# bogus2000/anytime-3D-reconstruction

Measured on AMD Instinct MI355X. Metric: 32^3 voxel reconstructions/sec at batch=256; IoU delta vs reference, higher is better.
Workload: dtype bf16

## Files before the change

### anytime-3d-reconstruction_amd/csrc/conv_direct.hip

```cpp
#include "direct_common.h"

namespace {

constexpr int CD_CIN = 64, CD_COUT = 128;
constexpr int CD_RB = CD_CIN * 2;
constexpr int CD_PIECES = 51;
constexpr int CD_TILE = CD_PIECES * 1024;
constexpr int CD_WST = CD_COUT * 128;
constexpr int CD_NST = 3;
constexpr int CD_RING = 2 * CD_TILE;
constexpr int CD_DUMMY = CD_RING + CD_NST * CD_WST;
constexpr int CD_LDS = CD_DUMMY + 1024;
constexpr int CD_SP = CD_COUT * 2 + 16;

__global__ __launch_bounds__(512, 1) void conv_direct_kernel(const __bf16 *__restrict__ x, const __bf16 *__restrict__ w,
                                                             const float *__restrict__ scale, const float *__restrict__ shift,
                                                             void *__restrict__ y, int dout_log2, unsigned x_bytes, unsigned w_bytes,
                                                             int act, int out_fp8) {
    extern __shared__ __attribute__((aligned(16))) char smem[];
    const int tid = threadIdx.x, lane = tid & 63;
    const int wave = __builtin_amdgcn_readfirstlane(tid >> 6);
    const int wm = wave >> 1, wn = wave & 1;
    const int lo = dout_log2, no = 1 << lo, li = lo + 1, n = 1 << li;

    const VvDirectBox box = vv_direct_box(no);
    const int b = box.b, od0 = box.od0, oh0 = box.oh0, ow0 = box.ow0;

    const u32x4 rsx = vv_make_rsrc(x, x_bytes), rsw = vv_make_rsrc(w, w_bytes);
    const unsigned lds0 = (unsigned)(unsigned long long)(lptr_t)smem;

    auto issue_x = [&](int q, int slot) {
        const int piece = slot * 8 + wave;
        const int rl = piece * 8 + (lane >> 3);
        const int zd = rl / 81, rem = rl - zd * 81, jh = rem / 9, jw = rem - jh * 9;
        const int g = (lane & 7) ^ (jw & 7);
        const int id = 2 * (od0 + zd) + ((q >> 2) & 1) - 1, ih = 2 * (oh0 + jh) + ((q >> 1) & 1) - 1, iw = 2 * (ow0 + jw) + (q & 1) - 1;
        const bool ok = q < 8 && rl < 405 && (unsigned)id < (unsigned)n && (unsigned)ih < (unsigned)n && (unsigned)iw < (unsigned)n;
        const unsigned vo = ok ? (unsigned)((((((b << li) + id) << li) + ih) << li) + iw) * CD_RB + g * 16 : 0xFFFFFFF0u;
        const unsigned dst = piece < CD_PIECES ? lds0 + (q & 1) * CD_TILE + piece * 1024 : lds0 + CD_DUMMY;
        vv_dma16(rsx, vo, dst);
    };
    auto issue_w = [&](int c) {
        const int q = c >> 3, a = c & 7;
        const int td = 2 * ((a >> 2) & 1) + ((q >> 2) & 1), th = 2 * ((a >> 1) & 1) + ((q >> 1) & 1), tw = 2 * (a & 1) + (q & 1);
        const int t = (td * 4 + th) * 4 + tw;
        const unsigned st = lds0 + CD_RING + (c % CD_NST) * CD_WST;
#pragma unroll
        for (int i = 0; i < 2; ++i) {
            const int row = (wave * 2 + i) * 8 + (lane >> 3);
            const int g = (lane & 7) ^ ((row >> 1) & 7);
            const unsigned vo = c < 64 ? (unsigned)row * (64 * CD_RB) + t * CD_RB + g * 16 : 0xFFFFFFF0u;
            vv_dma16(rsw, vo, st + (wave * 2 + i) * 1024);
        }
    };

#pragma unroll 1
    for (int s = 0; s < 7; ++s) issue_x(0, s);
    issue_w(0);
    issue_w(1);
    issue_w(2);
    vv_wait_vm<0>();
    __syncthreads();

    const int fr = lane & 31, fh = lane >> 5;
    const int rl0 = wm * 81 + (fr >> 3) * 9 + (fr & 7);
    unsigned xo[2][4], wo[4];
#pragma unroll
    for (int aw = 0; aw < 2; ++aw)
#pragma unroll
        for (int ks = 0; ks < 4; ++ks) xo[aw][ks] = lds0 + rl0 * CD_RB + (((ks * 2 + fh) ^ (((fr & 7) + aw) & 7)) << 4);
#pragma unroll
    for (int ks = 0; ks < 4; ++ks) wo[ks] = lds0 + CD_RING + (wn * 64 + fr) * 128 + (((ks * 2 + fh) ^ ((fr >> 1) & 7)) << 4);

    f32x16 acc[2][2];
#pragma unroll
    for (int i = 0; i < 2; ++i)
#pragma unroll
        for (int j = 0; j < 2; ++j)
#pragma unroll
            for (int e = 0; e < 16; ++e) acc[i][j][e] = 0.f;

#define CD_LDFRAG(F, XA, XOFF, WA)                                                                                              \
    asm volatile("ds_read_b128 %0, %4 offset:%6\n\tds_read_b128 %1, %4 offset:%7\n\tds_read_b128 %2, %5\n\tds_read_b128 %3, %5 offset:4096" \
                 : "=&v"(F[0]), "=&v"(F[1]), "=&v"(F[2]), "=&v"(F[3])                                                           \
                 : "v"(XA), "v"(WA), "n"(XOFF), "n"((XOFF) + 4 * 9 * CD_RB)                                                    \
                 : "memory")
#define CD_WAITFRAG(F, N) asm volatile("s_waitcnt lgkmcnt(%4)" : "+v"(F[0]), "+v"(F[1]), "+v"(F[2]), "+v"(F[3]) : "n"(N) : "memory")
#define CD_MFMA4(F)                                                                                                             \
    do {                                                                                                                        \
        _Pragma("unroll") for (int nt = 0; nt < 2; ++nt) _Pragma("unroll") for (int mt = 0; mt < 2; ++mt)                       \
            acc[nt][mt] = __builtin_amdgcn_mfma_f32_32x32x16_bf16(*reinterpret_cast<const bf16x8 *>(&F[2 + nt]),                \
                                                                  *reinterpret_cast<const bf16x8 *>(&F[mt]), acc[nt][mt], 0, 0, 0); \
        __builtin_amdgcn_sched_barrier(0);                                                                                      \
    } while (0)

    u32x4 P[4], Q[4];
    CD_LDFRAG(P, xo[0][0], 0, wo[0]);

#pragma unroll 1
    for (int q = 0; q < 8; ++q) {
        const unsigned tsel = (q & 1) * CD_TILE, tnext = ((q + 1) & 1) * CD_TILE;
        auto tap = [&](auto a_c) {
            constexpr int A = decltype(a_c)::value;
            constexpr int AW = A & 1, TO = (((A >> 2) & 1) * 81 + ((A >> 1) & 1) * 9 + AW) * CD_RB;
            constexpr int AN = (A + 1) & 7, AWN = AN & 1, TON = (((AN >> 2) & 1) * 81 + ((AN >> 1) & 1) * 9 + AWN) * CD_RB;
            const int c = q * 8 + A;
            const unsigned wsel = (c % CD_NST) * CD_WST, wnext = ((c + 1) % CD_NST) * CD_WST;
            CD_LDFRAG(Q, xo[AW][1] + tsel, TO, wo[1] + wsel);
            CD_WAITFRAG(P, 4);
            CD_MFMA4(P);
            CD_LDFRAG(P, xo[AW][2] + tsel, TO, wo[2] + wsel);
            CD_WAITFRAG(Q, 4);
            CD_MFMA4(Q);
            CD_LDFRAG(Q, xo[AW][3] + tsel, TO, wo[3] + wsel);
            CD_WAITFRAG(P, 4);
            CD_MFMA4(P);
            CD_WAITFRAG(Q, 0);
            vv_wait_vm<(A == 0 || A == 7) ? 2 : 3>();
            __syncthreads();
            if (A < 7) issue_x(q + 1, A);
            issue_w(c + 3);
            CD_LDFRAG(P, xo[AWN][0] + (A == 7 ? tnext : tsel), TON, wo[0] + wnext);
            CD_MFMA4(Q);
        };
        tap(std::integral_constant<int, 0>{});
        tap(std::integral_constant<int, 1>{});
        tap(std::integral_constant<int, 2>{});
        tap(std::integral_constant<int, 3>{});
        tap(std::integral_constant<int, 4>{});
        tap(std::integral_constant<int, 5>{});
        tap(std::integral_constant<int, 6>{});
        tap(std::integral_constant<int, 7>{});
    }
    CD_WAITFRAG(P, 0);
    vv_wait_vm<0>();
    __syncthreads();

    char *stage = smem;
    f32x4 scv[2][4], shv[2][4];
#pragma unroll
    for (int nt = 0; nt < 2; ++nt)
#pragma unroll
        for (int g = 0; g < 4; ++g) { scv[nt][g] = f32x4{1.f, 1.f, 1.f, 1.f}; shv[nt][g] = f32x4{0.f, 0.f, 0.f, 0.f}; }
    if (scale) {
#pragma unroll
        for (int nt = 0; nt < 2; ++nt)
#pragma unroll
            for (int g = 0; g < 4; ++g) scv[nt][g] = *reinterpret_cast<const f32x4 *>(scale + wn * 64 + nt * 32 + 8 * g + 4 * fh);
    }
    if (shift) {
#pragma unroll
        for (int nt = 0; nt < 2; ++nt)
#pragma unroll
            for (int g = 0; g < 4; ++g) shv[nt][g] = *reinterpret_cast<const f32x4 *>(shift + wn * 64 + nt * 32 + 8 * g + 4 * fh);
    }
    auto fill = VV_DIRECT_FILL32(CD_SP, wn * 64);
    auto with_out = [&](auto act_c) {
        if (out_fp8) fill(act_c, std::true_type{});
        else fill(act_c, std::false_type{});
    };
    VV_WITH_ACT(act, with_out);
    __syncthreads();
    vv_direct_store_box<512, CD_SP, CD_COUT, CD_COUT>(stage, y, box, lo, tid, out_fp8);
}

__global__ __launch_bounds__(512, 1) void conv_direct16_kernel(const __bf16 *__restrict__ x, const __bf16 *__restrict__ w,
                                                             const float *__restrict__ scale, const float *__restrict__ shift,
                                                             void *__restrict__ y, int dout_log2, unsigned x_bytes, unsigned w_bytes,
                                                             int act, int out_fp8) {
    extern __shared__ __attribute__((aligned(16))) char smem[];
    const int tid = threadIdx.x, lane = tid & 63;
    const int wave = __builtin_amdgcn_readfirstlane(tid >> 6);
    const int wm = wave >> 1, wn = wave & 1;
    const int lo = dout_log2, no = 1 << lo, li = lo + 1, n = 1 << li;

    const VvDirectBox box = vv_direct_box(no);
    const int b = box.b, od0 = box.od0, oh0 = box.oh0, ow0 = box.ow0;

    const u32x4 rsx = vv_make_rsrc(x, x_bytes), rsw = vv_make_rsrc(w, w_bytes);
    const unsigned lds0 = (unsigned)(unsigned long long)(lptr_t)smem;

    auto issue_x = [&](int q, int slot) {
        const int piece = slot * 8 + wave;
        const int rl = piece * 8 + (lane >> 3);
        const int zd = rl / 81, rem = rl - zd * 81, jh = rem / 9, jw = rem - jh * 9;
        const int g = (lane & 7) ^ ((2 * jw) & 7);
        const int id = 2 * (od0 + zd) + ((q >> 2) & 1) - 1, ih = 2 * (oh0 + jh) + ((q >> 1) & 1) - 1, iw = 2 * (ow0 + jw) + (q & 1) - 1;
        const bool ok = q < 8 && rl < 405 && (unsigned)id < (unsigned)n && (unsigned)ih < (unsigned)n && (unsigned)iw < (unsigned)n;
        const unsigned vo = ok ? (unsigned)((((((b << li) + id) << li) + ih) << li) + iw) * CD_RB + g * 16 : 0xFFFFFFF0u;
        const unsigned dst = piece < CD_PIECES ? lds0 + (q & 1) * CD_TILE + piece * 1024 : lds0 + CD_DUMMY;
        vv_dma16(rsx, vo, dst);
    };
    auto issue_w = [&](int c) {
        const int q = c >> 3, a = c & 7;
        const int td = 2 * ((a >> 2) & 1) + ((q >> 2) & 1), th = 2 * ((a >> 1) & 1) + ((q >> 1) & 1), tw = 2 * (a & 1) + (q & 1);
        const int t = (td * 4 + th) * 4 + tw;
        const unsigned st = lds0 + CD_RING + (c % CD_NST) * CD_WST;
#pragma unroll
        for (int i = 0; i < 2; ++i) {
            const int row = (wave * 2 + i) * 8 + (lane >> 3);
            const int g = (lane & 7) ^ ((row >> 1) & 7);
            const unsigned vo = c < 64 ? (unsigned)row * (64 * CD_RB) + t * CD_RB + g * 16 : 0xFFFFFFF0u;
            vv_dma16(rsw, vo, st + (wave * 2 + i) * 1024);
        }
    };

#pragma unroll 1
    for (int s = 0; s < 7; ++s) issue_x(0, s);
    issue_w(0);
    issue_w(1);
    issue_w(2);
    vv_wait_vm<0>();
    __syncthreads();

    const int r = lane & 15, kq = lane >> 4;
    const int rl0 = wm * 81 + (r >> 3) * 9 + (r & 7);
    unsigned xo[2][2], wo[2];
#pragma unroll
    for (int aw = 0; aw < 2; ++aw)
#pragma unroll
        for (int ks = 0; ks < 2; ++ks) xo[aw][ks] = lds0 + rl0 * CD_RB + (((ks * 4 + kq) ^ ((2 * ((r & 7) + aw)) & 7)) << 4);
#pragma unroll
    for (int ks = 0; ks < 2; ++ks) wo[ks] = lds0 + CD_RING + (wn * 64 + r) * 128 + (((ks * 4 + kq) ^ ((r >> 1) & 7)) << 4);

    f32x4 acc[4][4];
#pragma unroll
    for (int i = 0; i < 4; ++i)
#pragma unroll
        for (int j = 0; j < 4; ++j) acc[i][j] = f32x4{0.f, 0.f, 0.f, 0.f};

#define CD16_LD(F, XA, XOFF, WA)                                                                                                    \
    asm volatile("ds_read_b128 %0, %8 offset:%10\n\tds_read_b128 %1, %8 offset:%11\n\tds_read_b128 %2, %8 offset:%12\n\t"         \
                 "ds_read_b128 %3, %8 offset:%13\n\tds_read_b128 %4, %9\n\tds_read_b128 %5, %9 offset:2048\n\t"                   \
                 "ds_read_b128 %6, %9 offset:4096\n\tds_read_b128 %7, %9 offset:6144"                                               \
                 : "=&v"(F[0]), "=&v"(F[1]), "=&v"(F[2]), "=&v"(F[3]), "=&v"(F[4]), "=&v"(F[5]), "=&v"(F[6]), "=&v"(F[7])            \
                 : "v"(XA), "v"(WA), "n"(XOFF), "n"((XOFF) + 2304), "n"((XOFF) + 4608), "n"((XOFF) + 6912)                          \
                 : "memory")
#define CD16_WAIT(F, N)                                                                                                             \
    asm volatile("s_waitcnt lgkmcnt(%8)"                                                                                            \
                 : "+v"(F[0]), "+v"(F[1]), "+v"(F[2]), "+v"(F[3]), "+v"(F[4]), "+v"(F[5]), "+v"(F[6]), "+v"(F[7])                    \
                 : "n"(N)                                                                                                           \
                 : "memory")
#define CD16_SB __builtin_amdgcn_sched_barrier(0)
#define CD16_RD(D, A, OFF) asm volatile("ds_read_b128 %0, %1 offset:%2" : "=&v"(D) : "v"(A), "n"(OFF) : "memory")
#define CD16_MF(F, COT, CT)                                                                                                         \
    acc[COT][CT] = __builtin_amdgcn_mfma_f32_16x16x32_bf16(*reinterpret_cast<const bf16x8 *>(&F[4 + COT]),                          \
                                                           *reinterpret_cast<const bf16x8 *>(&F[CT]), acc[COT][CT], 0, 0, 0)

    u32x4 P[8], Q[8];
    CD16_LD(P, xo[0][0], 0, wo[0]);

#pragma unroll 1
    for (int q = 0; q < 8; ++q) {
        const unsigned tsel = (q & 1) * CD_TILE, tnext = ((q + 1) & 1) * CD_TILE;
        auto tap = [&](auto a_c) {
            constexpr int A = decltype(a_c)::value;
            constexpr int AW = A & 1, TO = (((A >> 2) & 1) * 81 + ((A >> 1) & 1) * 9 + AW) * CD_RB;
            constexpr int AN = (A + 1) & 7, AWN = AN & 1, TON = (((AN >> 2) & 1) * 81 + ((AN >> 1) & 1) * 9 + AWN) * CD_RB;
            const int c = q * 8 + A;
            const unsigned wsel = (c % CD_NST) * CD_WST, wnext = ((c + 1) % CD_NST) * CD_WST;
            const unsigned xq = xo[AW][1] + tsel, wq = wo[1] + wsel;
            CD16_WAIT(P, 0);
            CD16_SB;
            CD16_MF(P, 0, 0); CD16_MF(P, 0, 1); CD16_SB; CD16_RD(Q[0], xq, TO); CD16_RD(Q[4], wq, 0); CD16_SB;
            CD16_MF(P, 0, 2); CD16_MF(P, 0, 3); CD16_SB; CD16_RD(Q[1], xq, TO + 2304); CD16_RD(Q[5], wq, 2048); CD16_SB;
            CD16_MF(P, 1, 0); CD16_MF(P, 1, 1); CD16_SB; CD16_RD(Q[2], xq, TO + 4608); CD16_RD(Q[6], wq, 4096); CD16_SB;
            CD16_MF(P, 1, 2); CD16_MF(P, 1, 3); CD16_SB; CD16_RD(Q[3], xq, TO + 6912); CD16_RD(Q[7], wq, 6144); CD16_SB;
            CD16_MF(P, 2, 0); CD16_MF(P, 2, 1); CD16_MF(P, 2, 2); CD16_MF(P, 2, 3);
            CD16_MF(P, 3, 0); CD16_MF(P, 3, 1); CD16_MF(P, 3, 2); CD16_MF(P, 3, 3);
            CD16_SB;
            CD16_WAIT(Q, 0);
            vv_wait_vm<(A == 0 || A == 7) ? 2 : 3>();
            __syncthreads();
            CD16_SB;
            CD16_MF(Q, 0, 0); CD16_MF(Q, 0, 1);
            if (A < 7) issue_x(q + 1, A);
            CD16_MF(Q, 0, 2); CD16_MF(Q, 0, 3);
            issue_w(c + 3);
            const unsigned xp = xo[AWN][0] + (A == 7 ? tnext : tsel), wp = wo[0] + wnext;
            CD16_SB;
            CD16_MF(Q, 1, 0); CD16_MF(Q, 1, 1); CD16_SB; CD16_RD(P[0], xp, TON); CD16_RD(P[4], wp, 0); CD16_SB;
            CD16_MF(Q, 1, 2); CD16_MF(Q, 1, 3); CD16_SB; CD16_RD(P[1], xp, TON + 2304); CD16_RD(P[5], wp, 2048); CD16_SB;
            CD16_MF(Q, 2, 0); CD16_MF(Q, 2, 1); CD16_SB; CD16_RD(P[2], xp, TON + 4608); CD16_RD(P[6], wp, 4096); CD16_SB;
            CD16_MF(Q, 2, 2); CD16_MF(Q, 2, 3); CD16_SB; CD16_RD(P[3], xp, TON + 6912); CD16_RD(P[7], wp, 6144); CD16_SB;
            CD16_MF(Q, 3, 0); CD16_MF(Q, 3, 1); CD16_MF(Q, 3, 2); CD16_MF(Q, 3, 3);
            CD16_SB;
        };
        tap(std::integral_constant<int, 0>{});
        tap(std::integral_constant<int, 1>{});
        tap(std::integral_constant<int, 2>{});
        tap(std::integral_constant<int, 3>{});
        tap(std::integral_constant<int, 4>{});
        tap(std::integral_constant<int, 5>{});
        tap(std::integral_constant<int, 6>{});
        tap(std::integral_constant<int, 7>{});
    }
    CD16_WAIT(P, 0);
    vv_wait_vm<0>();
    __syncthreads();

    char *stage = smem;
    f32x4 scv[4], shv[4];
#pragma unroll
    for (int cot = 0; cot < 4; ++cot) { scv[cot] = f32x4{1.f, 1.f, 1.f, 1.f}; shv[cot] = f32x4{0.f, 0.f, 0.f, 0.f}; }
    if (scale) {
#pragma unroll
        for (int cot = 0; cot < 4; ++cot) scv[cot] = *reinterpret_cast<const f32x4 *>(scale + wn * 64 + cot * 16 + 4 * kq);
    }
    if (shift) {
#pragma unroll
        for (int cot = 0; cot < 4; ++cot) shv[cot] = *reinterpret_cast<const f32x4 *>(shift + wn * 64 + cot * 16 + 4 * kq);
    }
    auto fill = VV_DIRECT_FILL16(CD_SP, wn * 64);
    auto with_out = [&](auto act_c) {
        if (out_fp8) fill(act_c, std::true_type{});
        else fill(act_c, std::false_type{});
    };
    VV_WITH_ACT(act, with_out);
    __syncthreads();
    vv_direct_store_box<512, CD_SP, CD_COUT, CD_COUT>(stage, y, box, lo, tid, out_fp8);
}


constexpr int CDH_COUT = 64;
constexpr int CDH_WST = CDH_COUT * 128;
constexpr int CDH_RING = CD_TILE;
constexpr int CDH_DUMMY = CDH_RING + CD_NST * CDH_WST;
constexpr int CDH_LDS = CDH_DUMMY + 1024;
constexpr int CDH_SP = CDH_COUT * 2 + 16;

__global__ __launch_bounds__(256, 2) void conv_direct16h_kernel(const __bf16 *__restrict__ x, const __bf16 *__restrict__ w,
                                                                const float *__restrict__ scale, const float *__restrict__ shift,
                                                                void *__restrict__ y, int dout_log2, unsigned x_bytes, unsigned w_bytes,
                                                                int act, int out_fp8, int stagger, int abl) {
    extern __shared__ __attribute__((aligned(16))) char smem[];
    const int tid = threadIdx.x, lane = tid & 63;
    const int wave = __builtin_amdgcn_readfirstlane(tid >> 6);
    const int wm = wave;
    const int lo = dout_log2, no = 1 << lo, li = lo + 1, n = 1 << li;

    const VvDirectBox box = vv_direct_box<true>(no);
    const int b = box.b, od0 = box.od0, oh0 = box.oh0, ow0 = box.ow0, nh = box.nh;

    const u32x4 rsx = vv_make_rsrc(x, x_bytes), rsw = vv_make_rsrc(w, w_bytes);
    const unsigned lds0 = (unsigned)(unsigned long long)(lptr_t)smem;

    auto issue_x = [&](int q, int slot) {
        const int piece = slot * 4 + wave;
        const int rl = piece * 8 + (lane >> 3);
        const int zd = rl / 81, rem = rl - zd * 81, jh = rem / 9, jw = rem - jh * 9;
        const int g = (lane & 7) ^ ((2 * jw) & 7);
        const int id = 2 * (od0 + zd) + ((q >> 2) & 1) - 1, ih = 2 * (oh0 + jh) + ((q >> 1) & 1) - 1, iw = 2 * (ow0 + jw) + (q & 1) - 1;
        const bool ok = rl < 405 && (unsigned)id < (unsigned)n && (unsigned)ih < (unsigned)n && (unsigned)iw < (unsigned)n;
        const unsigned vo = ok ? (unsigned)((((((b << li) + id) << li) + ih) << li) + iw) * CD_RB + g * 16 : 0xFFFFFFF0u;
        const unsigned dst = piece < CD_PIECES ? lds0 + piece * 1024 : lds0 + CDH_DUMMY;
        vv_dma16(rsx, vo, dst);
    };
    auto issue_w = [&](int c) {
        const int q = c >> 3, a = c & 7;
        const int td = 2 * ((a >> 2) & 1) + ((q >> 2) & 1), th = 2 * ((a >> 1) & 1) + ((q >> 1) & 1), tw = 2 * (a & 1) + (q & 1);
        const int t = (td * 4 + th) * 4 + tw;
        const unsigned st = lds0 + CDH_RING + (c % CD_NST) * CDH_WST;
#pragma unroll
        for (int i = 0; i < 2; ++i) {
            const int row = (wave * 2 + i) * 8 + (lane >> 3);
            const int g = (lane & 7) ^ ((row >> 1) & 7);
            const unsigned vo = c < 64 ? (unsigned)(nh * CDH_COUT + row) * (64 * CD_RB) + t * CD_RB + g * 16 : 0xFFFFFFF0u;
            vv_dma16(rsw, vo, st + (wave * 2 + i) * 1024);
        }
    };

    {
        unsigned hwid;
        asm volatile("s_getreg_b32 %0, hwreg(HW_REG_HW_ID)" : "=s"(hwid));
        if ((hwid & 1u) && stagger) {
            for (int i = 0; i < stagger; ++i) __builtin_amdgcn_s_sleep(8);
        }
    }
#pragma unroll 1
    for (int s = 0; s < 13; ++s) issue_x(0, s);
    issue_w(0);
    issue_w(1);
    issue_w(2);
    vv_wait_vm<0>();
    __syncthreads();

    const int r = lane & 15, kq = lane >> 4;
    const int rl0 = wm * 81 + (r >> 3) * 9 + (r & 7);
    unsigned xo[2][2], wo[2];
#pragma unroll
    for (int aw = 0; aw < 2; ++aw)
#pragma unroll
        for (int ks = 0; ks < 2; ++ks) xo[aw][ks] = lds0 + rl0 * CD_RB + (((ks * 4 + kq) ^ ((2 * ((r & 7) + aw)) & 7)) << 4);
#pragma unroll
    for (int ks = 0; ks < 2; ++ks) wo[ks] = lds0 + CDH_RING + r * 128 + (((ks * 4 + kq) ^ ((r >> 1) & 7)) << 4);

    f32x4 acc[4][4];
#pragma unroll
    for (int i = 0; i < 4; ++i)
#pragma unroll
        for (int j = 0; j < 4; ++j) acc[i][j] = f32x4{0.f, 0.f, 0.f, 0.f};

    u32x4 P[8], Q[8];
#pragma unroll 1
    for (int q = 0; q < 8; ++q) {
        if (q > 0) {
            vv_wait_vm<0>();
            __syncthreads();
        }
        CD16_LD(P, xo[0][0], 0, wo[0] + ((q * 8) % CD_NST) * CDH_WST);
        auto tap = [&](auto a_c) {
            constexpr int A = decltype(a_c)::value;
            constexpr int AW = A & 1, TO = (((A >> 2) & 1) * 81 + ((A >> 1) & 1) * 9 + AW) * CD_RB;
            constexpr int AN = (A + 1) & 7, AWN = AN & 1, TON = (((AN >> 2) & 1) * 81 + ((AN >> 1) & 1) * 9 + AWN) * CD_RB;
            const int c = q * 8 + A;
            const unsigned wsel = (c % CD_NST) * CDH_WST, wnext = ((c + 1) % CD_NST) * CDH_WST;
            const unsigned xq = xo[AW][1], wq = wo[1] + wsel;
            CD16_WAIT(P, 0);
            CD16_SB;
            CD16_MF(P, 0, 0); CD16_MF(P, 0, 1); CD16_SB; CD16_RD(Q[0], xq, TO); CD16_RD(Q[4], wq, 0); CD16_SB;
            CD16_MF(P, 0, 2); CD16_MF(P, 0, 3); CD16_SB; CD16_RD(Q[1], xq, TO + 2304); CD16_RD(Q[5], wq, 2048); CD16_SB;
            CD16_MF(P, 1, 0); CD16_MF(P, 1, 1); CD16_SB; CD16_RD(Q[2], xq, TO + 4608); CD16_RD(Q[6], wq, 4096); CD16_SB;
            CD16_MF(P, 1, 2); CD16_MF(P, 1, 3); CD16_SB; CD16_RD(Q[3], xq, TO + 6912); CD16_RD(Q[7], wq, 6144); CD16_SB;
            CD16_MF(P, 2, 0); CD16_MF(P, 2, 1); CD16_MF(P, 2, 2); CD16_MF(P, 2, 3);
            CD16_MF(P, 3, 0); CD16_MF(P, 3, 1); CD16_MF(P, 3, 2); CD16_MF(P, 3, 3);
            CD16_SB;
            CD16_WAIT(Q, 0);
            vv_wait_vm<2>();
            __syncthreads();
            CD16_SB;
            CD16_MF(Q, 0, 0); CD16_MF(Q, 0, 1);
            CD16_MF(Q, 0, 2); CD16_MF(Q, 0, 3);
            issue_w(c + 3);
            CD16_SB;
            if (A < 7) {
                const unsigned xp = xo[AWN][0], wp = wo[0] + wnext;
                CD16_MF(Q, 1, 0); CD16_MF(Q, 1, 1); CD16_SB; CD16_RD(P[0], xp, TON); CD16_RD(P[4], wp, 0); CD16_SB;
                CD16_MF(Q, 1, 2); CD16_MF(Q, 1, 3); CD16_SB; CD16_RD(P[1], xp, TON + 2304); CD16_RD(P[5], wp, 2048); CD16_SB;
                CD16_MF(Q, 2, 0); CD16_MF(Q, 2, 1); CD16_SB; CD16_RD(P[2], xp, TON + 4608); CD16_RD(P[6], wp, 4096); CD16_SB;
                CD16_MF(Q, 2, 2); CD16_MF(Q, 2, 3); CD16_SB; CD16_RD(P[3], xp, TON + 6912); CD16_RD(P[7], wp, 6144); CD16_SB;
            } else {
                const bool more = q < 7 && !(abl & 1);
                CD16_MF(Q, 1, 0); CD16_MF(Q, 1, 1); CD16_SB;
                if (more) { issue_x(q + 1, 0); issue_x(q + 1, 1); issue_x(q + 1, 2); }
                CD16_SB; CD16_MF(Q, 1, 2); CD16_MF(Q, 1, 3); CD16_SB;
                if (more) { issue_x(q + 1, 3); issue_x(q + 1, 4); issue_x(q + 1, 5); }
                CD16_SB; CD16_MF(Q, 2, 0); CD16_MF(Q, 2, 1); CD16_SB;
                if (more) { issue_x(q + 1, 6); issue_x(q + 1, 7); issue_x(q + 1, 8); }
                CD16_SB; CD16_MF(Q, 2, 2); CD16_MF(Q, 2, 3); CD16_SB;
                if (more) { issue_x(q + 1, 9); issue_x(q + 1, 10); issue_x(q + 1, 11); issue_x(q + 1, 12); }
                CD16_SB;
            }
            CD16_MF(Q, 3, 0); CD16_MF(Q, 3, 1); CD16_MF(Q, 3, 2); CD16_MF(Q, 3, 3);
            CD16_SB;
        };
        tap(std::integral_constant<int, 0>{});
        tap(std::integral_constant<int, 1>{});
        tap(std::integral_constant<int, 2>{});
        tap(std::integral_constant<int, 3>{});
        tap(std::integral_constant<int, 4>{});
        tap(std::integral_constant<int, 5>{});
        tap(std::integral_constant<int, 6>{});
        tap(std::integral_constant<int, 7>{});
    }
    vv_wait_vm<0>();
    __syncthreads();

    char *stage = smem;
    f32x4 scv[4], shv[4];
#pragma unroll
    for (int cot = 0; cot < 4; ++cot) { scv[cot] = f32x4{1.f, 1.f, 1.f, 1.f}; shv[cot] = f32x4{0.f, 0.f, 0.f, 0.f}; }
    if (scale) {
#pragma unroll
        for (int cot = 0; cot < 4; ++cot) scv[cot] = *reinterpret_cast<const f32x4 *>(scale + nh * CDH_COUT + cot * 16 + 4 * kq);
    }
    if (shift) {
#pragma unroll
        for (int cot = 0; cot < 4; ++cot) shv[cot] = *reinterpret_cast<const f32x4 *>(shift + nh * CDH_COUT + cot * 16 + 4 * kq);
    }
    auto fill = VV_DIRECT_FILL16(CDH_SP, 0);
    auto with_out = [&](auto act_c) {
        if (out_fp8) fill(act_c, std::true_type{});
        else fill(act_c, std::false_type{});
    };
    VV_WITH_ACT(act, with_out);
    __syncthreads();
    vv_direct_store_box<256, CDH_SP, CDH_COUT, CD_COUT>(stage, y, box, lo, tid, out_fp8);
}


}

VV_EXPORT int vv_conv3d_k4s2_direct_supported(int side, int cin, int cout, int dtype) {
    return dtype == VV_BF16 && cin == CD_CIN && cout == CD_COUT && side >= 16 && vv_is_pow2(side);
}

VV_EXPORT int vv_conv3d_k4s2_direct_fwd_io(const void *x, const void *w_packed, const float *scale, const float *shift, void *y,
                                           int batch, int side, int cin, int cout, int act, int dtype, int out_dtype, void *stream) {
    if (!x || !w_packed || !y) return VV_ERR_NULL;
    if (out_dtype != VV_BF16 && out_dtype != VV_FP8) return VV_ERR_DTYPE;
    if (!vv_conv3d_k4s2_direct_supported(side, cin, cout, dtype) || batch <= 0) return VV_ERR_SHAPE;
    if (!vv_aligned16(x) || !vv_aligned16(w_packed) || !vv_aligned16(y)) return VV_ERR_ALIGN;
    const int so = side / 2;
    const int boxes = (so / 4) * (so / 8) * (so / 8);
    vv_allow_lds<&conv_direct_kernel>(CD_LDS);
    vv_allow_lds<&conv_direct16_kernel>(CD_LDS);
    vv_allow_lds<&conv_direct16h_kernel>(CDH_LDS);
    const int shape = vv_hook_int(vv_hook("VV_CD_SHAPE"), 16);
    const bool s16 = shape != 32, half = shape == 8;
    const size_t in_per = (size_t)side * side * side * cin * 2, out_per = (size_t)so * so * so * cout * (out_dtype == VV_FP8 ? 1 : 2);
    const int per = vv_chunk_samples(in_per, batch);
    if (per < 1) return VV_ERR_SHAPE;
    for (int b0 = 0; b0 < batch; b0 += per) {
        const int nb = batch - b0 < per ? batch - b0 : per;
        const __bf16 *xc = reinterpret_cast<const __bf16 *>(reinterpret_cast<const char *>(x) + (size_t)b0 * in_per);
        void *yc = reinterpret_cast<char *>(y) + (size_t)b0 * out_per;
        if (half)
            VV_LAUNCH(conv_direct16h_kernel, dim3(nb * boxes * 2), dim3(256), CDH_LDS, reinterpret_cast<hipStream_t>(stream), xc,
                      reinterpret_cast<const __bf16 *>(w_packed), scale, shift, yc, vv_log2(so), (unsigned)((size_t)nb * in_per),
                      (unsigned)((size_t)64 * cin * cout * 2), act, out_dtype == VV_FP8 ? 1 : 0,
                      vv_hook_int(vv_hook("VV_CDH_STAGGER"), 5), vv_hook_int(vv_hook("VV_CDH_ABL"), 0));
        else if (s16)
            VV_LAUNCH(conv_direct16_kernel, dim3(nb * boxes), dim3(512), CD_LDS, reinterpret_cast<hipStream_t>(stream), xc,
                      reinterpret_cast<const __bf16 *>(w_packed), scale, shift, yc, vv_log2(so), (unsigned)((size_t)nb * in_per),
                      (unsigned)((size_t)64 * cin * cout * 2), act, out_dtype == VV_FP8 ? 1 : 0);
        else
            VV_LAUNCH(conv_direct_kernel, dim3(nb * boxes), dim3(512), CD_LDS, reinterpret_cast<hipStream_t>(stream), xc,
                      reinterpret_cast<const __bf16 *>(w_packed), scale, shift, yc, vv_log2(so), (unsigned)((size_t)nb * in_per),
                      (unsigned)((size_t)64 * cin * cout * 2), act, out_dtype == VV_FP8 ? 1 : 0);
        const int rc = vv_launch_status();
        if (rc != VV_OK) return rc;
    }
    return VV_OK;
}

VV_EXPORT int vv_conv3d_k4s2_direct_fwd(const void *x, const void *w_packed, const float *scale, const float *shift, void *y,
                                        int batch, int side, int cin, int cout, int act, int dtype, void *stream) {
    return vv_conv3d_k4s2_direct_fwd_io(x, w_packed, scale, shift, y, batch, side, cin, cout, act, dtype, dtype, stream);
}
```

### anytime-3d-reconstruction_amd/csrc/convt_whole.hip

```cpp

#include <utility>

#include "common.h"

namespace {

constexpr int CW_X = 512 * 256;
constexpr int CW_WST = 64 * 128;
constexpr int CW_NST = 3;
constexpr int CW_RING = CW_X;
constexpr int CW_ZERO = CW_RING + CW_NST * CW_WST;
constexpr int CW_SS = CW_ZERO + 256;
constexpr int CW_LDS = CW_SS + 512;

#define CW_LD(F, X0, X1, WA)                                                                                                     \
    asm volatile("ds_read_b128 %0, %4\n\tds_read_b128 %1, %5\n\tds_read_b128 %2, %6\n\tds_read_b128 %3, %6 offset:4096"          \
                 : "=&v"(F[0]), "=&v"(F[1]), "=&v"(F[2]), "=&v"(F[3])                                                            \
                 : "v"(X0), "v"(X1), "v"(WA)                                                                                     \
                 : "memory")
#define CW_WAIT(F, N) asm volatile("s_waitcnt lgkmcnt(%4)" : "+v"(F[0]), "+v"(F[1]), "+v"(F[2]), "+v"(F[3]) : "n"(N) : "memory")
#define CW_MFMA4(F)                                                                                                              \
    do {                                                                                                                         \
        _Pragma("unroll") for (int nt = 0; nt < 2; ++nt) _Pragma("unroll") for (int mt = 0; mt < 2; ++mt)                        \
            acc[nt][mt] = __builtin_amdgcn_mfma_f32_32x32x16_bf16(*reinterpret_cast<const bf16x8 *>(&F[2 + nt]),                 \
                                                                  *reinterpret_cast<const bf16x8 *>(&F[mt]), acc[nt][mt], 0, 0, 0); \
        __builtin_amdgcn_sched_barrier(0);                                                                                       \
    } while (0)

template <int ACT>
__global__ __launch_bounds__(512, 1) void ctw_kernel(const __bf16 *__restrict__ x, const __bf16 *__restrict__ w,
                                                     const float *__restrict__ scale, const float *__restrict__ shift,
                                                     __bf16 *__restrict__ y, int npar) {
    extern __shared__ __attribute__((aligned(256))) char smem[];
    const int tid = threadIdx.x, lane = tid & 63;
    const int wave = __builtin_amdgcn_readfirstlane(tid >> 6);
    const int ps = 8 / npar;
    const int b = (int)blockIdx.x / ps, p0 = ((int)blockIdx.x % ps) * npar;
    const int NC = npar * 16;
    const unsigned lds0 = (unsigned)(unsigned long long)(lptr_t)smem;

    const u32x4 rsx = vv_make_rsrc(x + (size_t)b * (512 * 128), CW_X);
    const u32x4 rsw = vv_make_rsrc(w, 64 * 128 * 64 * 2);

    {
        const int pos = lane & 15, vsub = lane >> 4;
#pragma unroll 1
        for (int i = 0; i < 16; ++i) {
            const int it = i * 8 + wave;
            const int v = it * 4 + vsub;
            vv_dma16(rsx, (unsigned)(v * 256 + ((pos ^ (v & 15)) << 4)), lds0 + it * 1024);
        }
    }
    const unsigned wv = (unsigned)((wave * 8 + (lane >> 3)) * 128 + (((lane & 7) ^ (((wave * 8 + (lane >> 3)) >> 1) & 7)) << 4));
    auto issue_w = [&](int c, int s) {
        const int cc = c < NC ? c : NC - 1;
        const unsigned soff = (unsigned)__builtin_amdgcn_readfirstlane((p0 * 16 + cc) * CW_WST);
        vv_dma16(rsw, wv, soff, lds0 + CW_RING + s * CW_WST + wave * 1024);
    };
    issue_w(0, 0);
    issue_w(1, 1);
    issue_w(2, 2);
    if (tid < 16) *reinterpret_cast<uint4 *>(smem + CW_ZERO + tid * 16) = uint4{0u, 0u, 0u, 0u};
    if (tid >= 64 && tid < 128) {
        const int ch = tid - 64;
        *reinterpret_cast<float *>(smem + CW_SS + ch * 4) = scale ? scale[ch] : 1.f;
        *reinterpret_cast<float *>(smem + CW_SS + 256 + ch * 4) = shift ? shift[ch] : 0.f;
    }
    vv_wait_vm<0>();
    __syncthreads();

    const int fr = lane & 31, fh = lane >> 5;
    const int mh = fr >> 3, mw = fr & 7;
    const unsigned wl = lds0 + CW_RING + fr * 128 + ((fh ^ ((fr >> 1) & 7)) << 4);
    const unsigned R0 = lds0 + (unsigned)((wave * 64 + mh * 8 + mw) << 8);
    const unsigned ZR = lds0 + CW_ZERO;
    const int cb = mh * 8 + mw;
    auto tap_setup = [&](auto a_c, int pd, int ph, int pw, unsigned &t0, unsigned &t1) {
        constexpr int A = decltype(a_c)::value;
        const int dd = pd - ((A >> 2) & 1), dh = ph - ((A >> 1) & 1), dw = pw - (A & 1);
        const bool okw = (unsigned)(wave + dd) < 8u && (unsigned)(mw + dw) < 8u;
        const int sft = dd * 64 + dh * 8 + dw;
        const unsigned key = ((unsigned)((cb + dh * 8 + dw) ^ fh) & 15u) << 4;
        const unsigned r0 = okw && (unsigned)(mh + dh) < 8u ? R0 + (unsigned)(sft << 8) : ZR;
        const unsigned r1 = okw && (unsigned)(mh + 4 + dh) < 8u ? R0 + (unsigned)((sft + 32) << 8) : ZR;
        t0 = r0 ^ key;
        t1 = r1 ^ key;
    };

    f32x16 acc[2][2];
#pragma unroll
    for (int i = 0; i < 2; ++i)
#pragma unroll
        for (int j = 0; j < 2; ++j)
#pragma unroll
            for (int e = 0; e < 16; ++e) acc[i][j][e] = 0.f;

    auto epilogue = [&](int p) {
        const int pd = (p >> 2) & 1, ph = (p >> 1) & 1, pw = p & 1;
        char *yb = reinterpret_cast<char *>(y) + ((((size_t)b * 16 + 2 * wave + pd) * 16) * 16) * 128 + fh * 16;
        const char *ss = smem + CW_SS + fh * 16;
#pragma unroll
        for (int nt = 0; nt < 2; ++nt) {
            u32x2 o[2][4];
#pragma unroll
            for (int g = 0; g < 4; ++g) {
                const f32x4 sc = *reinterpret_cast<const f32x4 *>(ss + (nt * 32 + 8 * g) * 4);
                const f32x4 sh = *reinterpret_cast<const f32x4 *>(ss + 256 + (nt * 32 + 8 * g) * 4);
#pragma unroll
                for (int mt = 0; mt < 2; ++mt) {
                    bf16x4 q;
#pragma unroll
                    for (int e = 0; e < 4; ++e) {
                        float t = acc[nt][mt][4 * g + e] * sc[e] + sh[e];
                        if (ACT == VV_ACT_ELU) { const float em = __expf(fminf(t, 0.f)) - 1.f; t = t > 0.f ? t : em; }
                        else if (ACT == VV_ACT_RELU) t = fmaxf(t, 0.f);
                        else if (ACT == VV_ACT_LRELU) t = t > 0.f ? t : 0.3f * t;
                        q[e] = static_cast<__bf16>(t);
                        acc[nt][mt][4 * g + e] = 0.f;
                    }
                    o[mt][g] = *reinterpret_cast<const u32x2 *>(&q);
                }
            }
#pragma unroll
            for (int mt = 0; mt < 2; ++mt) {
                char *row = yb + (size_t)(((2 * (mt * 4 + mh) + ph) * 16 + 2 * mw + pw) * 128) + nt * 64;
#pragma unroll
                for (int j = 0; j < 2; ++j) {
                    u32x2 lo = o[mt][2 * j], hi = o[mt][2 * j + 1];
                    auto rx = __builtin_amdgcn_permlane32_swap(lo[0], hi[0], false, false);
                    auto ry = __builtin_amdgcn_permlane32_swap(lo[1], hi[1], false, false);
                    *reinterpret_cast<u32x4 *>(row + j * 32) = u32x4{rx[0], ry[0], rx[1], ry[1]};
                }
            }
        }
    };

    u32x4 P[4], Q[4];
    unsigned ua0, ua1, ub0, ub1;
    tap_setup(std::integral_constant<int, 0>{}, (p0 >> 2) & 1, (p0 >> 1) & 1, p0 & 1, ua0, ua1);
    unsigned ws = wl;
    int stg = 0;
    int cw = 3;
    CW_LD(P, ua0, ua1, ws);
#pragma unroll 1
    for (int pi = 0; pi < npar; ++pi) {
        const int p = p0 + pi, pd = (p >> 2) & 1, ph = (p >> 1) & 1, pw = p & 1;
        const int pn = p + 1, pnd = (pn >> 2) & 1, pnh = (pn >> 1) & 1, pnw = pn & 1;
        auto chunk = [&](auto j_c) {
            constexpr int J = decltype(j_c)::value, A = J >> 1, KH = J & 1;
            const unsigned x0 = KH ? ua0 ^ 128u : ua0, x1 = KH ? ua1 ^ 128u : ua1;
            CW_LD(Q, x0 ^ 32u, x1 ^ 32u, ws ^ 32u);
            CW_WAIT(P, 4);
            CW_MFMA4(P);
            if (KH == 0) {
                if (A < 7) tap_setup(std::integral_constant<int, (A + 1) & 7>{}, pd, ph, pw, ub0, ub1);
                else tap_setup(std::integral_constant<int, 0>{}, pnd, pnh, pnw, ub0, ub1);
            }
            CW_LD(P, x0 ^ 64u, x1 ^ 64u, ws ^ 64u);
            CW_WAIT(Q, 4);
            CW_MFMA4(Q);
            CW_LD(Q, x0 ^ 96u, x1 ^ 96u, ws ^ 96u);
            CW_WAIT(P, 4);
            CW_MFMA4(P);
            CW_WAIT(Q, 0);
            if (J < 2 && pi > 0) vv_wait_vm<9>();
            else vv_wait_vm<1>();
            __builtin_amdgcn_s_barrier();
            issue_w(cw, stg);
            ++cw;
            stg = stg == CW_NST - 1 ? 0 : stg + 1;
            ws = wl + stg * CW_WST;
            if (KH == 0) {
                CW_LD(P, ua0 ^ 128u, ua1 ^ 128u, ws);
            } else {
                ua0 = ub0;
                ua1 = ub1;
                CW_LD(P, ua0, ua1, ws);
            }
            CW_MFMA4(Q);
        };
        chunk(std::integral_constant<int, 0>{});
        chunk(std::integral_constant<int, 1>{});
        chunk(std::integral_constant<int, 2>{});
        chunk(std::integral_constant<int, 3>{});
        chunk(std::integral_constant<int, 4>{});
        chunk(std::integral_constant<int, 5>{});
        chunk(std::integral_constant<int, 6>{});
        chunk(std::integral_constant<int, 7>{});
        chunk(std::integral_constant<int, 8>{});
        chunk(std::integral_constant<int, 9>{});
        chunk(std::integral_constant<int, 10>{});
        chunk(std::integral_constant<int, 11>{});
        chunk(std::integral_constant<int, 12>{});
        chunk(std::integral_constant<int, 13>{});
        chunk(std::integral_constant<int, 14>{});
        chunk(std::integral_constant<int, 15>{});
        epilogue(p);
    }
    CW_WAIT(P, 0);
    vv_wait_vm<0>();
}


#define CW16_LD(F, XA, WA)                                                                                                          \
    asm volatile("ds_read_b128 %0, %8\n\tds_read_b128 %1, %9\n\tds_read_b128 %2, %10\n\tds_read_b128 %3, %11\n\t"                    \
                 "ds_read_b128 %4, %12\n\tds_read_b128 %5, %12 offset:2048\n\tds_read_b128 %6, %12 offset:4096\n\t"                  \
                 "ds_read_b128 %7, %12 offset:6144"                                                                                 \
                 : "=&v"(F[0]), "=&v"(F[1]), "=&v"(F[2]), "=&v"(F[3]), "=&v"(F[4]), "=&v"(F[5]), "=&v"(F[6]), "=&v"(F[7])            \
                 : "v"(XA[0]), "v"(XA[1]), "v"(XA[2]), "v"(XA[3]), "v"(WA)                                                           \
                 : "memory")
#define CW16_WAIT(F, N)                                                                                                             \
    asm volatile("s_waitcnt lgkmcnt(%8)"                                                                                            \
                 : "+v"(F[0]), "+v"(F[1]), "+v"(F[2]), "+v"(F[3]), "+v"(F[4]), "+v"(F[5]), "+v"(F[6]), "+v"(F[7])                    \
                 : "n"(N)                                                                                                           \
                 : "memory")
#define CW16_SB __builtin_amdgcn_sched_barrier(0)
#define CW16_RD(D, A, OFF) asm volatile("ds_read_b128 %0, %1 offset:%2" : "=&v"(D) : "v"(A), "n"(OFF) : "memory")
#define CW16_MF(F, COT, CT)                                                                                                         \
    acc[COT][CT] = __builtin_amdgcn_mfma_f32_16x16x32_bf16(*reinterpret_cast<const bf16x8 *>(&F[4 + COT]),                          \
                                                           *reinterpret_cast<const bf16x8 *>(&F[CT]), acc[COT][CT], 0, 0, 0)

template <int ACT, bool STATS = false>
__global__ __launch_bounds__(512, 1) void ctw16_kernel(const __bf16 *__restrict__ x, const __bf16 *__restrict__ w,
                                                       const float *__restrict__ scale, const float *__restrict__ shift,
                                                       __bf16 *__restrict__ y, int npar, float *__restrict__ partial = nullptr) {
    extern __shared__ __attribute__((aligned(256))) char smem[];
    const int tid = threadIdx.x, lane = tid & 63;
    const int wave = __builtin_amdgcn_readfirstlane(tid >> 6);
    const int ps = 8 / npar;
    const int b = (int)blockIdx.x / ps, p0 = ((int)blockIdx.x % ps) * npar;
    const int NC = npar * 16;
    const unsigned lds0 = (unsigned)(unsigned long long)(lptr_t)smem;

    const u32x4 rsx = vv_make_rsrc(x + (size_t)b * (512 * 128), CW_X);
    const u32x4 rsw = vv_make_rsrc(w, 64 * 128 * 64 * 2);
    {
        const int pos = lane & 15, vsub = lane >> 4;
#pragma unroll 1
        for (int i = 0; i < 16; ++i) {
            const int it = i * 8 + wave;
            const int v = it * 4 + vsub;
            vv_dma16(rsx, (unsigned)(v * 256 + ((pos ^ ((2 * v) & 15)) << 4)), lds0 + it * 1024);
        }
    }
    const unsigned wv = (unsigned)((wave * 8 + (lane >> 3)) * 128 + (((lane & 7) ^ (((wave * 8 + (lane >> 3)) >> 1) & 7)) << 4));
    auto issue_w = [&](int c, int s) {
        const int cc = c < NC ? c : NC - 1;
        const unsigned soff = (unsigned)__builtin_amdgcn_readfirstlane((p0 * 16 + cc) * CW_WST);
        vv_dma16(rsw, wv, soff, lds0 + CW_RING + s * CW_WST + wave * 1024);
    };
    issue_w(0, 0);
    issue_w(1, 1);
    issue_w(2, 2);
    if (tid < 16) *reinterpret_cast<uint4 *>(smem + CW_ZERO + tid * 16) = uint4{0u, 0u, 0u, 0u};
    if (tid >= 64 && tid < 128) {
        const int ch = tid - 64;
        *reinterpret_cast<float *>(smem + CW_SS + ch * 4) = scale ? scale[ch] : 1.f;
        *reinterpret_cast<float *>(smem + CW_SS + 256 + ch * 4) = shift ? shift[ch] : 0.f;
    }
    vv_wait_vm<0>();
    __syncthreads();

    const int r = lane & 15, q = lane >> 4;
    const int rh = r >> 3, rw = r & 7;
    const unsigned wl = lds0 + CW_RING + r * 128 + ((q ^ ((r >> 1) & 7)) << 4);
    const unsigned R0 = lds0 + (unsigned)((wave * 64 + r) << 8);
    const unsigned ZR = lds0 + CW_ZERO;
    auto tap_setup = [&](auto a_c, int pd, int ph, int pw, unsigned (&t)[4]) {
        constexpr int A = decltype(a_c)::value;
        const int dd = pd - ((A >> 2) & 1), dh = ph - ((A >> 1) & 1), dw = pw - (A & 1);
        const bool okw = (unsigned)(wave + dd) < 8u && (unsigned)(rw + dw) < 8u;
        const int sft = dd * 64 + dh * 8 + dw;
        const unsigned key = ((unsigned)((2 * (rw + dw)) ^ q) & 15u) << 4;
#pragma unroll
        for (int ct = 0; ct < 4; ++ct) {
            const unsigned row = okw && (unsigned)(2 * ct + rh + dh) < 8u ? R0 + (unsigned)((sft + 16 * ct) << 8) : ZR;
            t[ct] = row ^ key;
        }
    };

    f32x4 acc[4][4];
#pragma unroll
    for (int i = 0; i < 4; ++i)
#pragma unroll
        for (int j = 0; j < 4; ++j) acc[i][j] = f32x4{0.f, 0.f, 0.f, 0.f};
    f32x4 st1[4], st2[4];
#pragma unroll
    for (int i = 0; i < 4; ++i) { st1[i] = f32x4{0.f, 0.f, 0.f, 0.f}; st2[i] = f32x4{0.f, 0.f, 0.f, 0.f}; }

    auto epilogue = [&](int p) {
        const int pd = (p >> 2) & 1, ph = (p >> 1) & 1, pw = p & 1;
        const int qo = (q & 1) * 32 + (q >> 1) * 16;
        char *yb = reinterpret_cast<char *>(y) + ((((size_t)b * 16 + 2 * wave + pd) * 16 + 2 * rh + ph) * 16 + 2 * rw + pw) * 128 + qo;
        const char *ss = smem + CW_SS + q * 16;
#pragma unroll
        for (int c2 = 0; c2 < 2; ++c2) {
            u32x2 o[2][4];
#pragma unroll
            for (int h = 0; h < 2; ++h) {
                const int cot = 2 * c2 + h;
                const f32x4 sc = *reinterpret_cast<const f32x4 *>(ss + cot * 64);
                const f32x4 sh = *reinterpret_cast<const f32x4 *>(ss + 256 + cot * 64);
#pragma unroll
                for (int ct = 0; ct < 4; ++ct) {
                    const f32x4 t = vv_bn_act4<ACT>(acc[cot][ct], sc, sh);
                    bf16x4 v;
#pragma unroll
                    for (int e = 0; e < 4; ++e) v[e] = static_cast<__bf16>(t[e]);
                    if (STATS) {
                        const f32x4 f = {(float)v[0], (float)v[1], (float)v[2], (float)v[3]};
                        st1[cot] += f;
                        st2[cot] += f * f;
                    }
                    acc[cot][ct] = f32x4{0.f, 0.f, 0.f, 0.f};
                    o[h][ct] = *reinterpret_cast<const u32x2 *>(&v);
                }
            }
#pragma unroll
            for (int ct = 0; ct < 4; ++ct) {
                auto rx = __builtin_amdgcn_permlane16_swap(o[0][ct][0], o[1][ct][0], false, false);
                auto ry = __builtin_amdgcn_permlane16_swap(o[0][ct][1], o[1][ct][1], false, false);
                *reinterpret_cast<u32x4 *>(yb + (size_t)(ct * 4 * 16 * 128) + c2 * 64) = u32x4{rx[0], ry[0], rx[1], ry[1]};
            }
        }
    };

    u32x4 P[8], Q[8];
    unsigned ua[4], ub[4];
    tap_setup(std::integral_constant<int, 0>{}, (p0 >> 2) & 1, (p0 >> 1) & 1, p0 & 1, ua);
    unsigned ws = wl;
    int stg = 0, cw = 3;
    CW16_LD(P, ua, ws);
#pragma unroll 1
    for (int pi = 0; pi < npar; ++pi) {
        const int p = p0 + pi, pd = (p >> 2) & 1, ph = (p >> 1) & 1, pw = p & 1;
        const int pn = p + 1, pnd = (pn >> 2) & 1, pnh = (pn >> 1) & 1, pnw = pn & 1;
        auto chunk = [&](auto j_c) {
            constexpr int J = decltype(j_c)::value, A = J >> 1, KH = J & 1;
            unsigned xq[4];
#pragma unroll
            for (int ct = 0; ct < 4; ++ct) xq[ct] = ua[ct] ^ (KH ? 192u : 64u);
            const unsigned wq = ws ^ 64u;
            CW16_WAIT(P, 0);
            CW16_SB;
            CW16_MF(P, 0, 0); CW16_MF(P, 0, 1); CW16_SB; CW16_RD(Q[0], xq[0], 0); CW16_RD(Q[4], wq, 0); CW16_SB;
            CW16_MF(P, 0, 2); CW16_MF(P, 0, 3); CW16_SB; CW16_RD(Q[1], xq[1], 0); CW16_RD(Q[5], wq, 2048); CW16_SB;
            CW16_MF(P, 1, 0); CW16_MF(P, 1, 1); CW16_SB; CW16_RD(Q[2], xq[2], 0); CW16_RD(Q[6], wq, 4096); CW16_SB;
            CW16_MF(P, 1, 2); CW16_MF(P, 1, 3); CW16_SB; CW16_RD(Q[3], xq[3], 0); CW16_RD(Q[7], wq, 6144); CW16_SB;
            CW16_MF(P, 2, 0); CW16_MF(P, 2, 1); CW16_MF(P, 2, 2); CW16_MF(P, 2, 3);
            if (KH == 0) {
                if (A < 7) tap_setup(std::integral_constant<int, (A + 1) & 7>{}, pd, ph, pw, ub);
                else tap_setup(std::integral_constant<int, 0>{}, pnd, pnh, pnw, ub);
            }
            CW16_MF(P, 3, 0); CW16_MF(P, 3, 1); CW16_MF(P, 3, 2); CW16_MF(P, 3, 3);
            CW16_SB;
            CW16_WAIT(Q, 0);
            if (J < 2 && pi > 0) vv_wait_vm<9>();
            else vv_wait_vm<1>();
            __builtin_amdgcn_s_barrier();
            CW16_SB;
            CW16_MF(Q, 0, 0); CW16_MF(Q, 0, 1); CW16_SB;
            issue_w(cw, stg);
            ++cw;
            stg = stg == CW_NST - 1 ? 0 : stg + 1;
            ws = wl + stg * CW_WST;
            if (KH == 0) {
#pragma unroll
                for (int ct = 0; ct < 4; ++ct) xq[ct] = ua[ct] ^ 128u;
            } else {
#pragma unroll
                for (int ct = 0; ct < 4; ++ct) xq[ct] = ua[ct] = ub[ct];
            }
            CW16_SB;
            CW16_MF(Q, 0, 2); CW16_MF(Q, 0, 3); CW16_SB; CW16_RD(P[0], xq[0], 0); CW16_RD(P[4], ws, 0); CW16_SB;
            CW16_MF(Q, 1, 0); CW16_MF(Q, 1, 1); CW16_SB; CW16_RD(P[1], xq[1], 0); CW16_RD(P[5], ws, 2048); CW16_SB;
            CW16_MF(Q, 1, 2); CW16_MF(Q, 1, 3); CW16_SB; CW16_RD(P[2], xq[2], 0); CW16_RD(P[6], ws, 4096); CW16_SB;
            CW16_MF(Q, 2, 0); CW16_MF(Q, 2, 1); CW16_SB; CW16_RD(P[3], xq[3], 0); CW16_RD(P[7], ws, 6144); CW16_SB;
            CW16_MF(Q, 2, 2); CW16_MF(Q, 2, 3);
            CW16_MF(Q, 3, 0); CW16_MF(Q, 3, 1); CW16_MF(Q, 3, 2); CW16_MF(Q, 3, 3);
            CW16_SB;
        };
        chunk(std::integral_constant<int, 0>{});
        chunk(std::integral_constant<int, 1>{});
        chunk(std::integral_constant<int, 2>{});
        chunk(std::integral_constant<int, 3>{});
        chunk(std::integral_constant<int, 4>{});
        chunk(std::integral_constant<int, 5>{});
        chunk(std::integral_constant<int, 6>{});
        chunk(std::integral_constant<int, 7>{});
        chunk(std::integral_constant<int, 8>{});
        chunk(std::integral_constant<int, 9>{});
        chunk(std::integral_constant<int, 10>{});
        chunk(std::integral_constant<int, 11>{});
        chunk(std::integral_constant<int, 12>{});
        chunk(std::integral_constant<int, 13>{});
        chunk(std::integral_constant<int, 14>{});
        chunk(std::integral_constant<int, 15>{});
        epilogue(p);
    }
    CW16_WAIT(P, 0);
    vv_wait_vm<0>();
    if (STATS) {
#pragma unroll
        for (int cot = 0; cot < 4; ++cot)
#pragma unroll
            for (int e = 0; e < 4; ++e) {
                float a = st1[cot][e], b2 = st2[cot][e];
#pragma unroll
                for (int o = 8; o > 0; o >>= 1) { a += __shfl_xor(a, o, 64); b2 += __shfl_xor(b2, o, 64); }
                st1[cot][e] = a; st2[cot][e] = b2;
            }
        __syncthreads();
        float *red = reinterpret_cast<float *>(smem);
        if (r == 0) {
#pragma unroll
            for (int cot = 0; cot < 4; ++cot) {
                *reinterpret_cast<f32x4 *>(red + (wave * 2 + 0) * 64 + 16 * cot + 4 * q) = st1[cot];
                *reinterpret_cast<f32x4 *>(red + (wave * 2 + 1) * 64 + 16 * cot + 4 * q) = st2[cot];
            }
        }
        __syncthreads();
        if (tid < 128) {
            const int which = tid >> 6, ch = tid & 63;
            float sacc = 0.f;
#pragma unroll
            for (int wv_ = 0; wv_ < 8; ++wv_) sacc += red[(wv_ * 2 + which) * 64 + ch];
            partial[((size_t)blockIdx.x * 2 + which) * 64 + ch] = sacc;
        }
    }
}


#ifndef C4_ABL
#define C4_ABL 0
#endif
template <int N, class Fn, int... I>
__device__ __forceinline__ void c4_static_for_impl(Fn &&fn, std::integer_sequence<int, I...>) {
    (fn(std::integral_constant<int, I>{}), ...);
}
template <int N, class Fn>
__device__ __forceinline__ void c4_static_for(Fn &&fn) {
    c4_static_for_impl<N>(fn, std::make_integer_sequence<int, N>{});
}
#define C4_SB __builtin_amdgcn_sched_barrier(0)
#define C4_RD(D, A, OFF) asm volatile("ds_read_b128 %0, %1 offset:%2" : "=&v"(D) : "v"(A), "n"(OFF) : "memory")
#define C4_WAIT(F)                                                                                                                  \
    asm volatile("s_waitcnt lgkmcnt(0)"                                                                                             \
                 : "+v"(F[0]), "+v"(F[1]), "+v"(F[2]), "+v"(F[3]), "+v"(F[4]), "+v"(F[5]), "+v"(F[6]), "+v"(F[7]), "+v"(F[8]),       \
                   "+v"(F[9]), "+v"(F[10]), "+v"(F[11])                                                                             \
                 :                                                                                                                  \
                 : "memory")

template <int ACT>
__global__ __launch_bounds__(256, 1) void ctw4_kernel(const __bf16 *__restrict__ x, const __bf16 *__restrict__ w,
                                                      const float *__restrict__ scale, const float *__restrict__ shift,
                                                      __bf16 *__restrict__ y, int npar) {
    extern __shared__ __attribute__((aligned(256))) char smem[];
    const int tid = threadIdx.x, lane = tid & 63;
    const int wave = __builtin_amdgcn_readfirstlane(tid >> 6);
    const int ps = 8 / npar;
    const int b = (int)blockIdx.x / ps, p0 = ((int)blockIdx.x % ps) * npar;
    const int NC = npar * 16;
    const unsigned lds0 = (unsigned)(unsigned long long)(lptr_t)smem;

    const u32x4 rsx = vv_make_rsrc(x + (size_t)b * (512 * 128), CW_X);
    const u32x4 rsw = vv_make_rsrc(w, 64 * 128 * 64 * 2);
    const __amdgpu_buffer_rsrc_t rsy = __builtin_amdgcn_make_buffer_rsrc(y + (size_t)b * (4096 * 64), 0, 4096 * 64 * 2, 0x00020000);
    {
        const int pos = lane & 15, vsub = lane >> 4;
#pragma unroll 1
        for (int i = 0; i < 32; ++i) {
            const int it = i * 4 + wave;
            const int v = it * 4 + vsub;
            vv_dma16(rsx, (unsigned)(v * 256 + ((pos ^ ((2 * v) & 15)) << 4)), lds0 + it * 1024);
        }
    }
    const int wr0 = wave * 16 + (lane >> 3), wr1 = wr0 + 8;
    const unsigned wv0 = (unsigned)(wr0 * 128 + (((lane & 7) ^ ((wr0 >> 1) & 7)) << 4));
    const unsigned wv1 = (unsigned)(wr1 * 128 + (((lane & 7) ^ ((wr1 >> 1) & 7)) << 4));
    auto issue_w = [&](int c, int s) {
        const int cc = c < NC ? c : NC - 1;
        const unsigned soff = (unsigned)__builtin_amdgcn_readfirstlane((p0 * 16 + cc) * CW_WST);
        vv_dma16(rsw, wv0, soff, lds0 + CW_RING + s * CW_WST + wave * 2048);
        vv_dma16(rsw, wv1, soff, lds0 + CW_RING + s * CW_WST + wave * 2048 + 1024);
    };
    issue_w(0, 0);
    issue_w(1, 1);
    issue_w(2, 2);
    if (tid < 16) *reinterpret_cast<uint4 *>(smem + CW_ZERO + tid * 16) = uint4{0u, 0u, 0u, 0u};

    const int r = lane & 15, q = lane >> 4;
    const int rh = r >> 3, rw = r & 7;
    if (tid >= 64 && tid < 128) {
        const int ch = tid - 64;
        *reinterpret_cast<float *>(smem + CW_SS + ch * 4) = scale ? scale[ch] : 1.f;
        *reinterpret_cast<float *>(smem + CW_SS + 256 + ch * 4) = shift ? shift[ch] : 0.f;
    }
    vv_wait_vm<0>();
    __syncthreads();
    u32x4 bss[4];
    const unsigned ssa = lds0 + CW_SS + q * 16;
    auto load_ss = [](auto c2_c, u32x4(&d)[4], unsigned a) {
        constexpr int C2 = decltype(c2_c)::value;
        C4_RD(d[0], a, C2 * 128);
        C4_RD(d[1], a, C2 * 128 + 64);
        C4_RD(d[2], a, 256 + C2 * 128);
        C4_RD(d[3], a, 256 + C2 * 128 + 64);
    };
    load_ss(std::integral_constant<int, 0>{}, bss, ssa);
    asm volatile("s_waitcnt lgkmcnt(0)" : "+v"(bss[0]), "+v"(bss[1]), "+v"(bss[2]), "+v"(bss[3]) : : "memory");

    const unsigned wl = lds0 + CW_RING + r * 128 + ((q ^ ((r >> 1) & 7)) << 4);
    const unsigned R0 = lds0 + (unsigned)((wave * 128 + r) << 8);
    const unsigned ZR = lds0 + CW_ZERO;
    unsigned tr0[2], tzr[2];
    bool tokw[2], tokwh[2];
    auto parity_setup = [&](int ph, int pw) {
#pragma unroll
        for (int aw = 0; aw < 2; ++aw) {
            const int dw = pw - aw;
            const unsigned key = ((unsigned)((2 * (rw + dw)) ^ q) & 15u) << 4;
            tr0[aw] = R0 ^ key;
            tzr[aw] = ZR ^ key;
            tokw[aw] = (unsigned)(rw + dw) < 8u;
            tokwh[aw] = tokw[aw] & (ph ? rh == 0 : rh == 1);
        }
    };
    auto tap_setup2 = [&](auto a_c, auto ct0_c, int pd, int ph, int pw, unsigned (&t)[8]) {
        constexpr int A = decltype(a_c)::value, CT0 = decltype(ct0_c)::value, AD = (A >> 2) & 1, AH = (A >> 1) & 1, AW = A & 1;
        const int dd = pd - AD, dh = ph - AH, dw = pw - AW;
        const int sft = (dd * 64 + dh * 8 + dw) << 8;
#pragma unroll
        for (int ct = CT0; ct < CT0 + 2; ++ct) {
            const bool plane = (unsigned)(2 * wave + (ct >> 2) + dd) < 8u;
            const bool special = ph ? (AH == 0 && (ct & 3) == 3) : (AH == 1 && (ct & 3) == 0);
            const bool ok = (special ? tokwh[AW] : tokw[AW]) & plane;
            t[ct] = ok ? tr0[AW] + (unsigned)(sft + ct * 4096) : tzr[AW];
        }
    };
    auto tap_setup = [&](auto a_c, int pd, int ph, int pw, unsigned (&t)[8]) {
        tap_setup2(a_c, std::integral_constant<int, 0>{}, pd, ph, pw, t);
        tap_setup2(a_c, std::integral_constant<int, 2>{}, pd, ph, pw, t);
        tap_setup2(a_c, std::integral_constant<int, 4>{}, pd, ph, pw, t);
        tap_setup2(a_c, std::integral_constant<int, 6>{}, pd, ph, pw, t);
    };

    f32x4 accA[4][8], accB[4][8];
    u32x4 P[12], Q[12];
    unsigned ua[8], ub[8];
    unsigned ws = wl;
    int stg = 0, cw = 3;

    float st_t[2] = {0.f, 0.f}, st_m[2] = {0.f, 0.f}, st_u[2] = {0.f, 0.f}, st_r[2][4] = {{0.f, 0.f, 0.f, 0.f}, {0.f, 0.f, 0.f, 0.f}};
    float av[2][4] = {{0.f, 0.f, 0.f, 0.f}, {0.f, 0.f, 0.f, 0.f}};
#define C4_ACCRD(D, SRC) asm volatile("v_accvgpr_read_b32 %0, %1" : "=v"(D) : "a"(SRC))
    u32x2 eo[2] = {u32x2{0u, 0u}, u32x2{0u, 0u}};
    unsigned yvo = 0;
    auto epi_gap = [&](auto &PREV, auto u_c, auto g_c, auto tail_c) {
        constexpr int U = decltype(u_c)::value, G = decltype(g_c)::value, C2 = U >> 3, CT = U & 7;
        constexpr bool TAIL = decltype(tail_c)::value;
        if constexpr (G < 28 && (C4_ABL & 512)) {
            constexpr int E = G / 7, S = G % 7;
            if constexpr (S == 0) { st_r[0][E] = av[0][E]; st_r[1][E] = av[1][E]; }
            asm volatile("v_fma_f32 %0, %0, %1, %2" : "+v"(st_t[0]) : "v"(st_u[0]), "v"(st_u[1]));
            asm volatile("v_fma_f32 %0, %0, %1, %2" : "+v"(st_t[1]) : "v"(st_u[0]), "v"(st_u[1]));
        } else
        if constexpr (G < 28) {
            constexpr int E = G / 7, S = G % 7;
#pragma unroll
            for (int h = 0; h < 2; ++h) {
                if constexpr (S == 0) {
                    if constexpr (U == 0) C4_ACCRD(av[h][E], PREV[2 * C2 + h][CT][E]);
                    st_t[h] = __builtin_fmaf(av[h][E], __builtin_bit_cast(f32x4, bss[h])[E], __builtin_bit_cast(f32x4, bss[2 + h])[E]);
                } else if constexpr (ACT == VV_ACT_ELU && !((C4_ABL & 32) && S < 6) && !((C4_ABL & 128) && S == 3)) {
                    if constexpr (S == 1) st_m[h] = fminf(st_t[h], 0.f);
                    else if constexpr (S == 2) st_m[h] = st_m[h] * 1.4426950408889634f;
                    else if constexpr (S == 3) st_m[h] = __builtin_amdgcn_exp2f(st_m[h]);
                    else if constexpr (S == 4) st_m[h] = st_m[h] - 1.f;
                    else if constexpr (S == 5) st_u[h] = fmaxf(st_t[h], 0.f);
                    else st_r[h][E] = st_u[h] + st_m[h];
                } else if constexpr (S == 6) {
                    if (ACT == VV_ACT_RELU) st_r[h][E] = fmaxf(st_t[h], 0.f);
                    else if (ACT == VV_ACT_LRELU) st_r[h][E] = st_t[h] > 0.f ? st_t[h] : 0.3f * st_t[h];
                    else st_r[h][E] = st_t[h];
                }
            }
        }
        if constexpr (G >= 28 && (C4_ABL & 64)) {
            if constexpr (G == 31) { eo[0][0] ^= __builtin_bit_cast(unsigned, st_r[0][0] + st_r[0][1] + st_r[0][2] + st_r[0][3]); eo[1][1] ^= __builtin_bit_cast(unsigned, st_r[1][0] + st_r[1][1] + st_r[1][2] + st_r[1][3] + av[0][0] + av[1][1]); }
        } else
        if constexpr (G >= 28 && U < 15) {
            constexpr int UN = U + 1, E = G - 28;
            C4_ACCRD(av[0][E], PREV[2 * (UN >> 3)][UN & 7][E]);
            C4_ACCRD(av[1][E], PREV[2 * (UN >> 3) + 1][UN & 7][E]);
        }
        if constexpr (C4_ABL & 64) {
        } else if constexpr (G == 28 || G == 29) {
            constexpr int e0 = 2 * (G - 28);
#pragma unroll
            for (int h = 0; h < 2; ++h) {
                typedef __attribute__((ext_vector_type(2))) __bf16 bf16x2;
                const bf16x2 v = {static_cast<__bf16>(st_r[h][e0]), static_cast<__bf16>(st_r[h][e0 + 1])};
                eo[h][G - 28] = __builtin_bit_cast(unsigned, v);
            }
        } else if constexpr (G == 30) {
            auto rx = __builtin_amdgcn_permlane16_swap(eo[0][0], eo[1][0], false, false);
            auto ry = __builtin_amdgcn_permlane16_swap(eo[0][1], eo[1][1], false, false);
            eo[0] = u32x2{rx[0], ry[0]};
            eo[1] = u32x2{rx[1], ry[1]};
        } else if constexpr (G == 31) {
            constexpr int UO = (CT >> 2) * (2 * 16 * 16 * 128) + (CT & 3) * (4 * 16 * 128) + C2 * 64;
            __builtin_amdgcn_raw_buffer_store_b128(u32x4{eo[0][0], eo[0][1], eo[1][0], eo[1][1]}, rsy, yvo, UO, 0);
            if constexpr (CT == 7 && !(TAIL && C2 == 1)) {
                load_ss(std::integral_constant<int, 1 - C2>{}, bss, ssa);
                if constexpr (TAIL) asm volatile("s_waitcnt lgkmcnt(0)" : "+v"(bss[0]), "+v"(bss[1]), "+v"(bss[2]), "+v"(bss[3]) : : "memory");
            }
        }
    };
    auto set_yvo = [&](int p) {
        const int pd = (p >> 2) & 1, ph = (p >> 1) & 1, pw = p & 1;
        yvo = (unsigned)(((((4 * wave + pd) * 16 + 2 * rh + ph) * 16 + 2 * rw + pw) * 128) + (q & 1) * 32 + (q >> 1) * 16);
    };

    auto kstep = [&](auto &ACC, u32x4(&F)[12], u32x4(&G)[12], const unsigned(&xa)[8], auto kx_c, unsigned wa, auto first_c, auto &&slot) {
        constexpr unsigned KX = (unsigned)decltype(kx_c)::value;
        constexpr bool FIRST = decltype(first_c)::value;
        unsigned ra[2] = {0u, 0u};
        c4_static_for<32>([&](auto i_c) {
            constexpr int i = decltype(i_c)::value, cot = i >> 3, ct = i & 7;
            if constexpr (C4_ABL & 16) {
                if constexpr (FIRST) ACC[cot][ct] = f32x4{0.f, 0.f, 0.f, 0.f};
            } else if constexpr (FIRST)
                ACC[cot][ct] = __builtin_amdgcn_mfma_f32_16x16x32_bf16(*reinterpret_cast<const bf16x8 *>(&F[8 + cot]), *reinterpret_cast<const bf16x8 *>(&F[ct]),
                                                                       f32x4{0.f, 0.f, 0.f, 0.f}, 0, 0, 0);
            else
                ACC[cot][ct] = __builtin_amdgcn_mfma_f32_16x16x32_bf16(*reinterpret_cast<const bf16x8 *>(&F[8 + cot]), *reinterpret_cast<const bf16x8 *>(&F[ct]),
                                                                       ACC[cot][ct], 0, 0, 0);
            C4_SB;
            if constexpr (C4_ABL & 8) {
            } else if constexpr (i <= 12) {
                if constexpr (i >= 1 && i <= 8) C4_RD(G[i - 1], ra[(i - 1) & 1], 0);
                else if constexpr (i >= 9) C4_RD(G[i - 1], wa, (i - 9) * 2048);
                if constexpr (i < 8) ra[i & 1] = xa[i] ^ KX;
            }
            if constexpr (i >= 13) slot(std::integral_constant<int, i - 13>{});
            C4_SB;
        });
    };

    auto parity_body = [&](auto set_c, auto epi_c, int pi) {
        constexpr int SET = decltype(set_c)::value;
        constexpr bool EPI = decltype(epi_c)::value;
        auto &ACC = *(SET ? &accB : &accA);
        auto &PREV = *(SET ? &accA : &accB);
        const int p = p0 + pi, pd = (p >> 2) & 1, ph = (p >> 1) & 1, pw = p & 1;
        const int pn = p + 1, pnd = (pn >> 2) & 1, pnh = (pn >> 1) & 1, pnw = pn & 1;
        if (EPI) set_yvo(p - 1);
        c4_static_for<16>([&](auto j_c) {
            constexpr int J = decltype(j_c)::value, A = J >> 1, KH = J & 1;
            C4_WAIT(P);
            C4_SB;
            kstep(ACC, P, Q, ua, std::integral_constant<int, KH ? 192 : 64>{}, ws ^ 64u, std::integral_constant<bool, J == 0>{}, [&](auto sl_c) {
                if constexpr (EPI && !(C4_ABL & 1)) epi_gap(PREV, j_c, sl_c, std::false_type{});
            });
            C4_WAIT(Q);
            if (EPI && J >= 2 && !(C4_ABL & 1)) vv_wait_vm<4>();
            else vv_wait_vm<2>();
            if constexpr (!(C4_ABL & 2)) __builtin_amdgcn_s_barrier();
            C4_SB;
            if constexpr (!(C4_ABL & 4)) issue_w(cw, stg);
            ++cw;
            stg = stg == CW_NST - 1 ? 0 : stg + 1;
            ws = wl + stg * CW_WST;
            if (KH == 1) {
#pragma unroll
                for (int ct = 0; ct < 8; ++ct) ua[ct] = ub[ct];
            }
            C4_SB;
            kstep(ACC, Q, P, ua, std::integral_constant<int, KH ? 0 : 128>{}, ws, std::false_type{}, [&](auto sl_c) {
                constexpr int sl = decltype(sl_c)::value;
                if constexpr (EPI && sl < 13 && !(C4_ABL & 1)) epi_gap(PREV, j_c, std::integral_constant<int, 19 + sl>{}, std::false_type{});
                if constexpr (KH == 0 && sl >= 13 && sl < 17) {
                    if constexpr (A < 7) {
                        tap_setup2(std::integral_constant<int, (A + 1) & 7>{}, std::integral_constant<int, 2 * (sl - 13)>{}, pd, ph, pw, ub);
                    } else {
                        if constexpr (sl == 13) parity_setup(pnh, pnw);
                        tap_setup2(std::integral_constant<int, 0>{}, std::integral_constant<int, 2 * (sl - 13)>{}, pnd, pnh, pnw, ub);
                    }
                }
            });
        });
    };

    parity_setup((p0 >> 1) & 1, p0 & 1);
    tap_setup(std::integral_constant<int, 0>{}, (p0 >> 2) & 1, (p0 >> 1) & 1, p0 & 1, ua);
#pragma unroll
    for (int k = 0; k < 8; ++k) C4_RD(P[k], ua[k], 0);
    C4_RD(P[8], ws, 0);
    C4_RD(P[9], ws, 2048);
    C4_RD(P[10], ws, 4096);
    C4_RD(P[11], ws, 6144);
    parity_body(std::integral_constant<int, 0>{}, std::false_type{}, 0);
#pragma unroll 1
    for (int pi = 1; pi < npar; pi += 2) {
        parity_body(std::integral_constant<int, 1>{}, std::true_type{}, pi);
        if (pi + 1 < npar) parity_body(std::integral_constant<int, 0>{}, std::true_type{}, pi + 1);
    }
    C4_WAIT(P);
    set_yvo(p0 + npar - 1);
    if ((npar - 1) & 1) {
        c4_static_for<16>([&](auto u_c) { c4_static_for<32>([&](auto k_c) { epi_gap(accB, u_c, k_c, std::true_type{}); }); });
    } else {
        c4_static_for<16>([&](auto u_c) { c4_static_for<32>([&](auto k_c) { epi_gap(accA, u_c, k_c, std::true_type{}); }); });
    }
    vv_wait_vm<0>();
}


}

VV_EXPORT int vv_convT3d_k4s2_whole_supported(int side, int cin, int cout, int dtype) {
    return dtype == VV_BF16 && side == 8 && cin == 128 && cout == 64;
}

VV_EXPORT int vv_convT3d_k4s2_whole_fwd(const void *x, const void *w_skip, const float *scale, const float *shift, void *y, int batch,
                                        int side, int cin, int cout, int act, int dtype, void *stream) {
    if (!x || !w_skip || !y) return VV_ERR_NULL;
    if (!vv_convT3d_k4s2_whole_supported(side, cin, cout, dtype) || batch <= 0) return VV_ERR_SHAPE;
    if (!vv_aligned16(x) || !vv_aligned16(w_skip) || !vv_aligned16(y)) return VV_ERR_ALIGN;
    int ps = 1;
    while (ps < 8 && (long)batch * ps < 256) ps *= 2;
    if (const char *e = vv_hook("VV_CTW_PS")) {
        const int v = atoi(e);
        if (v == 1 || v == 2 || v == 4 || v == 8) ps = v;
    }
    const int shape = vv_hook_int(vv_hook("VV_CTW_SHAPE"), 16);
    const bool shape16 = shape != 32;
    hipStream_t st = reinterpret_cast<hipStream_t>(stream);
    auto launch = [&](auto act_c) {
        constexpr int ACT = decltype(act_c)::value;
        vv_allow_lds<&ctw_kernel<ACT>>(CW_LDS);
        vv_allow_lds<&ctw16_kernel<ACT>>(CW_LDS);
        vv_allow_lds<&ctw4_kernel<ACT>>(CW_LDS);
        if (shape != 16 && shape != 32)
            VV_LAUNCH(ctw4_kernel<ACT>, dim3((unsigned)batch * ps), dim3(256), CW_LDS, st, reinterpret_cast<const __bf16 *>(x),
                      reinterpret_cast<const __bf16 *>(w_skip), scale, shift, reinterpret_cast<__bf16 *>(y), 8 / ps);
        else if (shape16)
            VV_LAUNCH(ctw16_kernel<ACT>, dim3((unsigned)batch * ps), dim3(512), CW_LDS, st, reinterpret_cast<const __bf16 *>(x),
                      reinterpret_cast<const __bf16 *>(w_skip), scale, shift, reinterpret_cast<__bf16 *>(y), 8 / ps);
        else
            VV_LAUNCH(ctw_kernel<ACT>, dim3((unsigned)batch * ps), dim3(512), CW_LDS, st, reinterpret_cast<const __bf16 *>(x),
                      reinterpret_cast<const __bf16 *>(w_skip), scale, shift, reinterpret_cast<__bf16 *>(y), 8 / ps);
    };
    vv_with_act(act, launch);
    return vv_launch_status();
}

VV_EXPORT int vv_convT3d_k4s2_whole_stats_blocks(int batch) { return batch > 0 ? batch : 0; }

VV_EXPORT int vv_convT3d_k4s2_whole_stats_fwd(const void *x, const void *w_skip, void *y, float *stats_partial, size_t stats_bytes, int batch,
                                              int side, int cin, int cout, int dtype, void *stream) {
    if (!x || !w_skip || !y || !stats_partial) return VV_ERR_NULL;
    if (!vv_convT3d_k4s2_whole_supported(side, cin, cout, dtype) || batch <= 0) return VV_ERR_SHAPE;
    if (!vv_aligned16(x) || !vv_aligned16(w_skip) || !vv_aligned16(y) || !vv_aligned16(stats_partial)) return VV_ERR_ALIGN;
    if (stats_bytes < (size_t)batch * 2 * 64 * sizeof(float)) return VV_ERR_WORKSPACE;
    vv_allow_lds<&ctw16_kernel<VV_ACT_NONE, true>>(CW_LDS);
    VV_LAUNCH((ctw16_kernel<VV_ACT_NONE, true>), dim3((unsigned)batch), dim3(512), CW_LDS, reinterpret_cast<hipStream_t>(stream),
              reinterpret_cast<const __bf16 *>(x), reinterpret_cast<const __bf16 *>(w_skip), nullptr, nullptr, reinterpret_cast<__bf16 *>(y), 8,
              stats_partial);
    return vv_launch_status();
}
```

### anytime-3d-reconstruction_amd/csrc/direct_common.h

```cpp
#pragma once
#include "common.h"

struct VvDirectBox { int b, od0, oh0, ow0, nh; };

template <bool HALVES = false>
__device__ __forceinline__ VvDirectBox vv_direct_box(int no) {
    const int nwg = gridDim.x;
    int blk = (nwg & 7) == 0 ? (int)(blockIdx.x & 7) * (nwg >> 3) + (int)(blockIdx.x >> 3) : (int)blockIdx.x;
    VvDirectBox o;
    o.nh = 0;
    if (HALVES) { o.nh = blk & 1; blk >>= 1; }
    const int bxw = no >> 3, bxh = no >> 3, bxd = no >> 2;
    const int bw = blk % bxw; blk /= bxw;
    const int bh = blk % bxh; blk /= bxh;
    const int bd = blk % bxd;
    o.b = blk / bxd;
    o.od0 = bd * 4; o.oh0 = bh * 8; o.ow0 = bw * 8;
    return o;
}

#define VV_DIRECT_PUT4(dst, c, v)                                                                          \
    do {                                                                                                   \
        if (FP8) {                                                                                         \
            *reinterpret_cast<unsigned *>(dst + c) = vv_pack_fp8x4(v);                                     \
        } else {                                                                                           \
            bf16x4 o;                                                                                      \
            _Pragma("unroll") for (int e = 0; e < 4; ++e) o[e] = static_cast<__bf16>(v[e]);                \
            *reinterpret_cast<bf16x4 *>(dst + c * 2) = o;                                                  \
        }                                                                                                  \
    } while (0)

#define VV_DIRECT_FILL16(PITCH, C0)                                                                        \
    [&](auto act_c, auto fp8_c) {                                                                          \
        constexpr int ACT = decltype(act_c)::value;                                                        \
        constexpr bool FP8 = decltype(fp8_c)::value;                                                       \
        _Pragma("unroll") for (int ct = 0; ct < 4; ++ct)                                                   \
            _Pragma("unroll") for (int cot = 0; cot < 4; ++cot) {                                          \
                const int c = (C0) + cot * 16 + 4 * kq;                                                    \
                const f32x4 sc = scv[cot], sh = shv[cot];                                                  \
                const f32x4 v = vv_bn_act4<ACT>(acc[cot][ct], sc, sh);                                     \
                char *dst = stage + (wm * 64 + ct * 16 + r) * (PITCH);                                     \
                VV_DIRECT_PUT4(dst, c, v);                                                                 \
            }                                                                                              \
    }
#define VV_DIRECT_FILL32(PITCH, C0)                                                                        \
    [&](auto act_c, auto fp8_c) {                                                                          \
        constexpr int ACT = decltype(act_c)::value;                                                        \
        constexpr bool FP8 = decltype(fp8_c)::value;                                                       \
        _Pragma("unroll") for (int mt = 0; mt < 2; ++mt)                                                   \
            _Pragma("unroll") for (int nt = 0; nt < 2; ++nt)                                               \
                _Pragma("unroll") for (int g = 0; g < 4; ++g) {                                            \
                    const int c = (C0) + nt * 32 + 8 * g + 4 * fh;                                         \
                    const f32x4 sc = scv[nt][g], sh = shv[nt][g];                                          \
                    f32x4 v;                                                                               \
                    _Pragma("unroll") for (int e = 0; e < 4; ++e) {                                        \
                        float t = acc[nt][mt][4 * g + e] * sc[e] + sh[e];                                  \
                        if (ACT == VV_ACT_ELU) { const float em = __expf(fminf(t, 0.f)) - 1.f; t = t > 0.f ? t : em; } \
                        else if (ACT == VV_ACT_RELU) t = fmaxf(t, 0.f);                                    \
                        else if (ACT == VV_ACT_LRELU) t = t > 0.f ? t : 0.3f * t;                          \
                        v[e] = t;                                                                          \
                    }                                                                                      \
                    char *dst = stage + (wm * 64 + mt * 32 + fr) * (PITCH);                                \
                    VV_DIRECT_PUT4(dst, c, v);                                                             \
                }                                                                                          \
    }

template <int THREADS, int PITCH, int STAGE_CH, int Y_CH>
__device__ __forceinline__ void vv_direct_store_box(const char *stage, void *y, const VvDirectBox &box, int lo, int tid, int out_fp8) {
    const int es = out_fp8 ? 1 : 2;
    const int cpr = STAGE_CH * es / 16;
    for (int id = tid; id < 256 * cpr; id += THREADS) {
        const int r = id / cpr, cc = id % cpr;
        const int od = box.od0 + (r >> 6), oh = box.oh0 + ((r >> 3) & 7), ow = box.ow0 + (r & 7);
        const size_t vox = ((((((size_t)box.b << lo) + od) << lo) + oh) << lo) + ow;
        *reinterpret_cast<uint4 *>(reinterpret_cast<char *>(y) + vox * (Y_CH * es) + box.nh * STAGE_CH * es + cc * 16) =
            *reinterpret_cast<const uint4 *>(stage + r * PITCH + cc * 16);
    }
}
```

### anytime-3d-reconstruction_amd/voxvae/lib.py

```python
import ctypes
import os

import torch

PKG = os.path.dirname(os.path.dirname(os.path.abspath(__file__)))
LIB_PATH = os.path.join(PKG, 'lib', 'libvoxvae.so')
HOOKS_LIB_PATH = os.path.join(PKG, 'lib', 'libvoxvae_hooks.so')
HOOK_VARS = ('VV_CD_SHAPE', 'VV_CDH_STAGGER', 'VV_CDH_ABL', 'VV_DIRECT_MT', 'VV_LT_KSLICE', 'VV_SPLIT_TARGET', 'VV_SPLIT_MINCHUNKS', 'VV_NO_KHALVES', 'VV_POSMAJOR_CONV_SIDE',
             'VV_POSMAJOR_CONVT_SIDE', 'VV_STAGES', 'VV_NO_FIRSTCONV', 'VV_WGRAD_F32', 'VV_PG_TARGET', 'VV_CTW_PS', 'VV_CTW_SHAPE',
             'VV_NO_WGRAD_PHASE', 'VV_BN_NB', 'VV_BN_SWEEP', 'VV_FINAL_BCE', 'VV_FIRSTCONV_GATHER', 'VV_FIRSTCONV_WGS', 'VV_FIRSTCONV_NOCHAIN', 'VV_CHUNK_SAMPLES')

VV_F32, VV_BF16, VV_FP8 = 0, 1, 2
ACT = {None: 0, 'None': 0, 'linear': 0, 'elu': 1, 'relu': 2, 'lrelu': 3}
DTYPES = {'f32': VV_F32, 'fp32': VV_F32, 'float32': VV_F32, 'bf16': VV_BF16, 'bfloat16': VV_BF16, 'fp8': VV_FP8}

_vp, _i, _f, _sz, _l = ctypes.c_void_p, ctypes.c_int, ctypes.c_float, ctypes.c_size_t, ctypes.c_long

SIGNATURES = {
    'vv_abi_version': (_i, []),
    'vv_status_string': (ctypes.c_char_p, [_i]),
    'vv_last_hip_error': (ctypes.c_char_p, []),
    'vv_pack_conv_k4': (_i, [_vp, _vp, _i, _i, _i, _vp]),
    'vv_pack_convT_k4s2': (_i, [_vp, _vp, _i, _i, _i, _vp]),
    'vv_pack_conv_k4s1_meanpool': (_i, [_vp, _vp, _i, _i, _i, _i, _vp]),
    'vv_pack_conv_k4s1_full': (_i, [_vp, _vp, _i, _i, _i, _i, _vp]),
    'vv_max_over_positions': (_i, [_vp, _vp, _i, _i, _i, _vp]),
    'vv_sigmoid_f32': (_i, [_vp, _vp, _l, _vp]),
    'vv_pack_convT_k4s1_dense': (_i, [_vp, _vp, _i, _i, _i, _i, _vp]),
    'vv_pack_dense': (_i, [_vp, _vp, _i, _i, _i, _vp]),
    'vv_fold_bn': (_i, [_vp, _vp, _vp, _vp, _vp, _f, _vp, _vp, _i, _i, _vp]),
    'vv_conv3d_first_fwd': (_i, [_vp, _vp, _vp, _vp, _vp, _i, _i, _i, _i, _i, _vp]),
    'vv_conv3d_first_fwd_io': (_i, [_vp, _vp, _vp, _vp, _vp, _i, _i, _i, _i, _i, _i, _vp]),
    'vv_conv3d_k4s2_workspace_bytes': (_sz, [_i, _i, _i, _i, _i]),
    'vv_conv3d_k4s2_fwd': (_i, [_vp, _vp, _vp, _vp, _vp, _i, _i, _i, _i, _i, _i, _vp, _sz, _vp]),
    'vv_convT3d_k4s2_workspace_bytes': (_sz, [_i, _i, _i, _i, _i]),
    'vv_convT3d_k4s2_fwd': (_i, [_vp, _vp, _vp, _vp, _vp, _i, _i, _i, _i, _i, _i, _vp, _sz, _vp]),
    'vv_conv3d_k4s2_fwd_io': (_i, [_vp, _vp, _vp, _vp, _vp, _i, _i, _i, _i, _i, _i, _i, _vp, _sz, _vp]),
    'vv_convT3d_k4s2_fwd_io': (_i, [_vp, _vp, _vp, _vp, _vp, _i, _i, _i, _i, _i, _i, _i, _vp, _sz, _vp]),
    'vv_conv3d_k4s2_direct_supported': (_i, [_i, _i, _i, _i]),
    'vv_conv3d_k4s2_direct_fwd': (_i, [_vp, _vp, _vp, _vp, _vp, _i, _i, _i, _i, _i, _i, _vp]),
    'vv_conv3d_k4s2_direct_fwd_io': (_i, [_vp, _vp, _vp, _vp, _vp, _i, _i, _i, _i, _i, _i, _i, _vp]),
    'vv_conv3d_k4s2_direct_fp8_supported': (_i, [_i, _i, _i]),
    'vv_conv3d_k4s2_direct_fp8_fwd': (_i, [_vp, _vp, _vp, _vp, _vp, _i, _i, _i, _i, _i, _i, _vp]),
    'vv_convT3d_k4s2_direct_supported': (_i, [_i, _i, _i, _i]),
    'vv_pack_convT_k4s2_frag': (_i, [_vp, _vp, _i, _i, _vp]),
    'vv_convT3d_k4s2_direct_fwd': (_i, [_vp, _vp, _vp, _vp, _vp, _i, _i, _i, _i, _i, _i, _vp]),
    'vv_convT3d_k4s2_direct_fp8_supported': (_i, [_i, _i, _i]),
    'vv_pack_convT_k4s2_frag_fp8': (_i, [_vp, _vp, _i, _i, _vp]),
    'vv_convT3d_k4s2_direct_fp8_fwd': (_i, [_vp, _vp, _vp, _vp, _vp, _i, _i, _i, _i, _i, _i, _vp]),
    'vv_conv3d_k4s2_skip_supported': (_i, [_i, _i, _i, _i]),
    'vv_convT3d_k4s2_skip_supported': (_i, [_i, _i, _i, _i]),
    'vv_pack_conv_k4_skip': (_i, [_vp, _vp, _i, _i, _vp]),
    'vv_pack_skip_images': (_i, [_vp, _vp, _vp, _vp, _vp, _i, _vp]),
    'vv_pack_convT_k4s2_skip': (_i, [_vp, _vp, _i, _i, _vp]),
    'vv_conv3d_k4s2_skip_fwd': (_i, [_vp, _vp, _vp, _vp, _vp, _i, _i, _i, _i, _i, _i, _vp]),
    'vv_convT3d_k4s2_skip_fwd': (_i, [_vp, _vp, _vp, _vp, _vp, _i, _i, _i, _i, _i, _i, _vp]),
    'vv_convT3d_k4s2_whole_supported': (_i, [_i, _i, _i, _i]),
    'vv_convT3d_k4s2_whole_fwd': (_i, [_vp, _vp, _vp, _vp, _vp, _i, _i, _i, _i, _i, _i, _vp]),
    'vv_conv3d_k4s2_pos_supported': (_i, [_i, _i, _i, _i]),
    'vv_convT3d_k4s2_pos_supported': (_i, [_i, _i, _i, _i]),
    'vv_conv3d_k4s2_pos_workspace_bytes': (_sz, [_i, _i, _i]),
    'vv_convT3d_k4s2_pos_workspace_bytes': (_sz, [_i, _i, _i]),
    'vv_conv3d_k4s2_pos_fwd': (_i, [_vp, _vp, _vp, _vp, _vp, _i, _i, _i, _i, _i, _i, _vp, _sz, _vp]),
    'vv_convT3d_k4s2_pos_fwd': (_i, [_vp, _vp, _vp, _vp, _vp, _i, _i, _i, _i, _i, _i, _vp, _sz, _vp]),
    'vv_dense_workspace_bytes': (_sz, [_i, _i, _i, _i]),
    'vv_dense_fwd': (_i, [_vp, _vp, _vp, _vp, _vp, _i, _i, _i, _i, _i, _i, _vp, _sz, _vp]),
    'vv_latent_tail_supported': (_i, [_i, _i, _i, _i, _i, _i, _i]),
    'vv_latent_tail_workspace_bytes': (_sz, [_i, _i, _i, _i]),
    'vv_latent_tail_fwd': (_i, [_vp] * 15 + [_i] * 9 + [_vp, _sz, _vp]),
    'vv_conv_pos_latent_tail_supported': (_i, [_i] * 8),
    'vv_conv_pos_latent_tail_workspace_bytes': (_sz, [_i, _i, _i, _i]),
    'vv_conv_pos_latent_tail_fwd': (_i, [_vp] * 4 + [_i, _i] + [_vp] * 14 + [_i] * 8 + [_vp, _sz, _vp]),
    'vv_reparam_kl_fwd': (_i, [_vp, _vp, _vp, _f, _vp, _vp, _i, _vp, _vp, _vp, _i, _i, _vp]),
    'vv_convT3d_final_bce_workspace_bytes': (_sz, [_i, _i]),
    'vv_convT3d_final_bce_fwd': (_i, [_vp, _vp, _vp, _vp, _vp, _vp, _i, _i, _i, _f, _f, _i, _vp, _sz, _vp]),
    'vv_convT3d_final_bce_metrics_fwd': (_i, [_vp, _vp, _vp, _vp, _vp, _vp, _vp, _i, _i, _i, _f, _f, _i, _vp, _sz, _vp]),
    'vv_shape_metrics': (_i, [_vp, _vp, _i, _vp]),
    'vv_sample_latents': (_i, [_vp, _vp, _vp, _vp, _vp, _i, _i, _i, _i, _vp]),
    'vv_convT3d_final_mean_workspace_bytes': (_sz, [_i, _i, _i]),
    'vv_convT3d_final_mean_fwd': (_i, [_vp, _vp, _vp, _vp, _vp, _i, _i, _i, _i, _f, _f, _i, _vp, _sz, _vp]),
    'vv_pr_curve_workspace_bytes': (_sz, [_i, _l, _i]),
    'vv_pr_curve_accumulate': (_i, [_vp, _vp, _i, _vp, _i, _i, _vp, _i, _vp, _vp, _vp, _sz, _i, _l, _vp]),
    'vv_voxel_points_workspace_bytes': (_sz, [_i, _i]),
    'vv_voxel_points_count': (_i, [_vp, _i, _f, _i, _i, _i, _vp, _vp, _vp, _vp, _sz, _vp]),
    'vv_voxel_points_emit': (_i, [_vp, _i, _f, _i, _vp, _vp, _vp, _vp, _vp, ctypes.c_longlong, _vp, _sz, _i, _i, _vp]),
    'vv_object_pose_workspace_bytes': (_sz, [_i]),
    'vv_object_pose': (_i, [_vp] * 4 + [_i, ctypes.c_double, ctypes.c_double] + [_vp] * 12 + [_sz, _vp]),
    'vv_object_pose_host': (_i, [_vp] * 4 + [_i, ctypes.c_double, ctypes.c_double] + [_vp] * 12 + [_i]),
    'vv_pose_translation_host': (_i, [_vp] * 7),
    'vv_pose_ray_host': (_i, [_vp, ctypes.c_double, ctypes.c_double, _vp]),
    'vv_pose_ray_rotation_host': (_i, [_vp, _vp]),
    'vv_pose_box_projection_host': (_i, [_vp, _vp, _vp, ctypes.c_double, ctypes.c_double, ctypes.c_double, _vp]),
    'vv_latent_mask_fill':(_i, [_vp, _vp, _vp, _i, _vp, _vp, _i, _i, _i, _vp]),
    'vv_nearest_category': (_i, [_vp, _vp, _vp, _i, _vp, _i, _i, _vp]),
    'vv_latent_correct': (_i, [_vp, _vp, _vp, _vp, _vp, _vp, _vp, _i, _i, _i, _vp]),
    'vv_category_accuracy': (_i, [_vp, _vp, _i, _vp, _i, _vp]),
    'vv_binary_loss': (_i, [_vp, _vp, _f, _f, _f, _vp, _i, ctypes.c_long, _vp]),
    'vv_voxel_precision_recall': (_i, [_vp, _vp, _f, _vp, _vp, _vp, _i, ctypes.c_long, _vp]),
    'vv_kl_loss': (_i, [_vp, _vp, _vp, _vp, _vp, _i, _i, _vp]),
    'vv_unpack_bits_gather': (_i, [_vp, _vp, _vp, _i, _l, _vp]),
    'vv_pack_bits': (_i, [_vp, _vp, _f, _l, _vp]),
    'vv_adam_step_multi': (_i, [_vp, _i, _f, _f, _f, _f, _vp]),
    'vv_convert': (_i, [_vp, _vp, _l, _i, _i, _vp]),
    'vv_regulizer_loss': (_i, [_vp, _vp, _vp, _f, _vp, _i, _i, _i, _vp]),
    'vv_sampling': (_i, [_vp, _vp, _vp, _vp, ctypes.c_long, _vp]),
    'vv_bn_workspace_bytes': (_sz, [_l, _i]),
    'vv_bn_train_stats': (_i, [_vp, _l, _i, _vp, _vp, _f, _f, _vp, _vp, _vp, _vp, _vp, _vp, _vp, _i, _vp, _sz, _vp]),
    'vv_bn_finalize_stats': (_i, [_vp, _i, _l, _i, _vp, _vp, _f, _f, _vp, _vp, _vp, _vp, _vp, _vp, _vp, _vp]),
    'vv_convT3d_k4s2_whole_stats_blocks': (_i, [_i]),
    'vv_convT3d_k4s2_whole_stats_fwd': (_i, [_vp, _vp, _vp, _vp, _sz, _i, _i, _i, _i, _i, _vp]),
    'vv_bn_act_fwd': (_i, [_vp, _vp, _vp, _vp, _l, _i, _i, _i, _vp]),
    'vv_bn_act_bwd': (_i, [_vp, _vp, _vp, _vp, _vp, _vp, _vp, _vp, _vp, _l, _i, _i, _i, _vp, _sz, _vp]),
    'vv_wgrad_workspace_bytes': (_sz, [_l, _i, _i]),
    'vv_wgrad_dense': (_i, [_vp, _vp, _vp, _l, _i, _i, _i, _i, _i, _vp, _sz, _vp]),
    'vv_wgrad_conv_k4s2': (_i, [_vp, _vp, _vp, _i, _i, _i, _i, _i, _i, _vp, _sz, _vp]),
    'vv_unpack_meanpool_grad': (_i, [_vp, _vp, _i, _i, _i, _vp]),
    'vv_unpack_convT_dense_grad': (_i, [_vp, _vp, _i, _i, _i, _vp]),
    'vv_transpose_f32': (_i, [_vp, _vp, _i, _i, _vp]),
    'vv_colsum': (_i, [_vp, _vp, _l, _i, _i, _vp]),
    'vv_bce_bwd': (_i, [_vp, _vp, _vp, _i, _l, _f, _f, _f, _vp]),
    'vv_reparam_kl_bwd': (_i, [_vp, _vp, _vp, _vp, _f, _vp, _i, _i, _f, _vp]),
    'vv_adam_step': (_i, [_vp, _vp, _vp, _vp, _l, _f, _f, _f, _f, _vp]),
}


class VoxVaeError(RuntimeError):
    pass


_lib = None
_hooks_lib = None


def _open(path, hooks):
    if not os.path.exists(path):
        raise VoxVaeError('HIP library missing: %s (run `python __graft_entry__.py` / voxvae/build.py); '
                          'there is no CPU fallback' % path)
    from . import build as _build
    if os.path.isdir(_build.CSRC) and os.path.exists(path + '.srchash') and not _build.is_current(hooks):
        raise VoxVaeError('%s is stale: csrc/ or include/voxvae.h changed since it was built (run `python __graft_entry__.py`)' % path)
    lib = ctypes.CDLL(path)
    for name, (res, args) in SIGNATURES.items():
        fn = getattr(lib, name)
        fn.restype, fn.argtypes = res, args
    return lib


def hooks_requested():
    env = os.environ
    return env.get('VOXVAE_TEST_HOOKS') == '1' and any(v in env for v in HOOK_VARS)


def load():
    global _lib, _hooks_lib
    if hooks_requested():
        if _hooks_lib is None:
            _hooks_lib = _open(HOOKS_LIB_PATH, True)
        return _hooks_lib
    if _lib is None:
        _lib = _open(LIB_PATH, False)
    return _lib


def check(status, what):
    if status != 0:
        detail = ' [%s]' % load().vv_last_hip_error().decode() if status == -6 else ''
        raise VoxVaeError('%s failed: %s (%d)%s' % (what, load().vv_status_string(status).decode(), status, detail))


def call(name, *args):
    check(getattr(load(), name)(*args), name)


def ptr(t):
    return None if t is None else ctypes.c_void_p(t.data_ptr())
```

### profiles/microbench/mb_ab_lib.py

```python
import ctypes, json, os, sys, time
import torch
_R = os.path.dirname(os.path.dirname(os.path.dirname(os.path.abspath(__file__)))); sys.path.insert(0, _R); sys.path.insert(0, os.path.join(_R, 'anytime-3d-reconstruction_amd'))
from voxvae import lib as L
other = sys.argv[2] if len(sys.argv) > 2 else 'base'
libs = {other: ctypes.CDLL(os.path.join(_R, sys.argv[1])), 'tree': L.load()}
hooks_libs = {other: ctypes.CDLL(os.path.join(_R, sys.argv[3])), 'tree': ctypes.CDLL(L.HOOKS_LIB_PATH)} if len(sys.argv) > 3 else None
if os.environ.get('AB_AA'):
    libs[other + '_aa'] = ctypes.CDLL(os.path.join(_R, os.environ['AB_AA']))
DEV = 'cuda:0'; B = 256
cs = ctypes.c_void_p(torch.cuda.current_stream().cuda_stream)
torch.manual_seed(0)
sc = torch.rand(256, device=DEV) + 0.5; sh = torch.randn(256, device=DEV) * 0.3


def bf(*shape):
    return torch.randn(*shape, device=DEV).to(torch.bfloat16)


def packed(fn, cin, cout, *extra):
    w = (torch.randn(4, 4, 4, cin, cout, device=DEV) / (8 * cin) ** 0.5).float().contiguous()
    o = torch.empty(64 * cin * cout, dtype=torch.bfloat16, device=DEV)
    L.call(fn, L.ptr(w), L.ptr(o), *extra, cs)
    return o


cases = {}
w = packed('vv_pack_convT_k4s2_skip', 64, 128, 128, 64)
x = bf(B, 8, 8, 8, 128)
cases['D4'] = ('vv_convT3d_k4s2_whole_fwd', lambda y: (L.ptr(x), L.ptr(w), L.ptr(sc), L.ptr(sh), L.ptr(y), B, 8, 128, 64, 1, L.VV_BF16, cs), (B, 16, 16, 16, 64))
w2 = packed('vv_pack_conv_k4', 64, 128, 64, 128, L.VV_BF16)
x2 = bf(B, 16, 16, 16, 64)
cases['E2'] = ('vv_conv3d_k4s2_direct_fwd', lambda y: (L.ptr(x2), L.ptr(w2), L.ptr(sc), L.ptr(sh), L.ptr(y), B, 16, 64, 128, 1, L.VV_BF16, cs), (B, 8, 8, 8, 128))
w3 = packed('vv_pack_conv_k4_skip', 128, 256, 128, 256)
x3 = bf(B, 8, 8, 8, 128)
cases['E3'] = ('vv_conv3d_k4s2_skip_fwd', lambda y: (L.ptr(x3), L.ptr(w3), L.ptr(sc), L.ptr(sh), L.ptr(y), B, 8, 128, 256, 1, L.VV_BF16, cs), (B, 4, 4, 4, 256))
w4 = packed('vv_pack_convT_k4s2_skip', 128, 256, 256, 128)
x4 = bf(B, 4, 4, 4, 256)
cases['D3'] = ('vv_convT3d_k4s2_skip_fwd', lambda y: (L.ptr(x4), L.ptr(w4), L.ptr(sc), L.ptr(sh), L.ptr(y), B, 4, 256, 128, 1, L.VV_BF16, cs), (B, 8, 8, 8, 128))

w2f = torch.empty(64 * 64 * 128, dtype=torch.uint8, device=DEV)
_w2 = (torch.randn(4, 4, 4, 64, 128, device=DEV) / 64).float().contiguous()
L.call('vv_pack_conv_k4', L.ptr(_w2), L.ptr(w2f), 64, 128, L.VV_FP8, cs)
x2f = torch.randn(B, 16, 16, 16, 64, device=DEV).to(torch.float8_e4m3fn)
cases['E2fp8'] = ('vv_conv3d_k4s2_direct_fp8_fwd', lambda y: (L.ptr(x2f), L.ptr(w2f), L.ptr(sc), L.ptr(sh), L.ptr(y), B, 16, 64, 128, 1, L.VV_BF16, cs), (B, 8, 8, 8, 128))
if hooks_libs:
    cases['E2s32'] = cases['E2'] + ({'VV_CD_SHAPE': '32'},)
    cases['E2h'] = cases['E2'] + ({'VV_CD_SHAPE': '8'},)


f32 = ctypes.c_float
timed = set(cases)
wk = (torch.randn(4, 4, 4, 1, 64, device=DEV) * 0.3).to(torch.bfloat16).float().contiguous()


def d5_case(dt, side, Bn):
    D = 2 * side
    xf = torch.randn(Bn, side, side, side, 64, device=DEV)
    xd = xf.contiguous() if dt == L.VV_F32 else xf.to(torch.bfloat16 if dt == L.VV_BF16 else torch.float8_e4m3fn)
    yd = (torch.rand(Bn, D, D, D, device=DEV) < 0.3).float()
    wsb = max(int(libs['tree'].vv_convT3d_final_bce_workspace_bytes(Bn, side)), 16)

    def mk():
        return {'probs': torch.full((Bn, D, D, D), -1.0, device=DEV), 'logits': torch.full((Bn, D, D, D), -1.0, device=DEV),
                'stats': torch.full((Bn, 4), -1.0, device=DEV), 'metrics': torch.full((4,), -1.0, device=DEV),
                '_ws': torch.empty(wsb, dtype=torch.uint8, device=DEV)}
    return ('vv_convT3d_final_bce_metrics_fwd', lambda o: (L.ptr(xd), L.ptr(wk), L.ptr(yd), L.ptr(o['probs']), L.ptr(o['logits']), L.ptr(o['stats']),
            L.ptr(o['metrics']), Bn, side, 64, f32(0.6), f32(1e-7), dt, L.ptr(o['_ws']), ctypes.c_size_t(wsb), cs), mk)


def mean_case(dt, Bn, K, side):
    D = 2 * side
    xf = torch.randn(Bn * K, side, side, side, 64, device=DEV)
    xd = xf.contiguous() if dt == L.VV_F32 else xf.to(torch.bfloat16)
    yd = (torch.rand(Bn, D, D, D, device=DEV) < 0.3).float()
    libs['tree'].vv_convT3d_final_mean_workspace_bytes.restype = ctypes.c_size_t
    wsb = max(int(libs['tree'].vv_convT3d_final_mean_workspace_bytes(Bn, K, side)), 16)

    def mk():
        return {'mean': torch.full((Bn, D, D, D), -1.0, device=DEV), 'stats': torch.full((Bn, 4), -1.0, device=DEV),
                '_ws': torch.empty(wsb, dtype=torch.uint8, device=DEV)}
    return ('vv_convT3d_final_mean_fwd', lambda o: (L.ptr(xd), L.ptr(wk), L.ptr(yd), L.ptr(o['mean']), L.ptr(o['stats']), Bn, K, side, 64,
            f32(0.6), f32(1e-7), dt, L.ptr(o['_ws']), ctypes.c_size_t(wsb), cs), mk)


def metrics_case(Bn):
    st = torch.cat([torch.rand(Bn, 1, device=DEV) * 900, torch.randint(0, 500, (Bn, 3), device=DEV).float()], 1).contiguous()
    return ('vv_shape_metrics', lambda o: (L.ptr(st), L.ptr(o['metrics']), Bn, cs), lambda: {'metrics': torch.full((4,), -1.0, device=DEV)})


def e1_case(Bn, side=32):
    xg = (torch.rand(Bn, side, side, side, device=DEV) < 0.3).float()
    w1 = packed('vv_pack_conv_k4', 1, 64, 1, 64, L.VV_BF16)
    h = side // 2
    return ('vv_conv3d_first_fwd_io', lambda o: (L.ptr(xg), L.ptr(w1), L.ptr(sc), L.ptr(sh), L.ptr(o['y']), Bn, side, 64, 1, L.VV_BF16, L.VV_BF16, cs),
            lambda: {'y': torch.full((Bn, h, h, h, 64), -1.0, dtype=torch.bfloat16, device=DEV)})


libs['tree'].vv_convT3d_final_bce_workspace_bytes.restype = ctypes.c_size_t
for side, Bn in ((8, 3), (16, 2)):
    cases['D5bf16_s%d' % side] = d5_case(L.VV_BF16, side, Bn)
    if hooks_libs:
        for form in ('box', 'sweep', 'sweepp'):
            cases['D5bf16_s%d_%s' % (side, form)] = cases['D5bf16_s%d' % side] + ({'VV_FINAL_BCE': form},)
cases['D5f32_s4'] = d5_case(L.VV_F32, 4, 3)
cases['D5f32_s32'] = d5_case(L.VV_F32, 32, 2)
cases['D5fp8_s8'] = d5_case(L.VV_FP8, 8, 3)
cases['D5mean_bf16_s8'] = mean_case(L.VV_BF16, 3, 8, 8)
cases['D5mean_bf16_s16'] = mean_case(L.VV_BF16, 2, 4, 16)
cases['D5mean_f32_s4'] = mean_case(L.VV_F32, 5, 3, 4)
cases['metrics_5'] = metrics_case(5)
cases['metrics_70'] = metrics_case(70)
cases['E1_B2'] = e1_case(2)
cases['E1_B64'] = e1_case(64)
cases['E1_B128'] = e1_case(128)
cases['D5fp8_256'] = d5_case(L.VV_FP8, 16, 256)
cases['D5mean_32x32'] = mean_case(L.VV_BF16, 32, 32, 16)
timed |= {'D5fp8_256', 'D5mean_32x32'}

only = os.environ.get('AB_ONLY', '').split(',') if os.environ.get('AB_ONLY') else list(cases)
N = 300
res = {}
release_libs = libs
for name in only:
    fn, args, oshape = cases[name][:3]
    env = cases[name][3] if len(cases[name]) > 3 else {}
    libs = hooks_libs if env else release_libs
    os.environ.update(env)
    ys = {k: oshape() if callable(oshape) else torch.empty(*oshape, dtype=torch.bfloat16, device=DEV) for k in libs}
    fs = {}
    for k in libs:
        f = getattr(libs[k], fn); f.restype = ctypes.c_int
        fs[k] = f
        assert f(*args(ys[k])) == 0
    torch.cuda.synchronize()
    if callable(oshape):
        same = all(bool(torch.equal(ys[other][n].view(torch.uint8), ys['tree'][n].view(torch.uint8))) for n in ys['tree'] if n[0] != '_')
    else:
        same = bool(torch.equal(ys[other], ys['tree']))
    t = {k: [] for k in libs}
    for rnd in range(4 if name in timed else 0):
        for k in libs:
            a = args(ys[k])
            for i in range(30):
                fs[k](*a)
            torch.cuda.synchronize()
            t0 = time.perf_counter()
            for i in range(N):
                fs[k](*a)
            torch.cuda.synchronize()
            t[k].append(1e6 * (time.perf_counter() - t0) / N)
    res[name] = {'bit_identical': same}
    if name in timed:
        res[name].update({'us_per_launch': {k: [round(v, 2) for v in t[k]] for k in libs}, 'tree_over_%s' % other: round(min(t['tree']) / min(t[other]), 4)})
        if other + '_aa' in libs:
            res[name]['%s_aa_over_%s' % (other, other)] = round(min(t[other + '_aa']) / min(t[other]), 4)
    for k in env:
        del os.environ[k]
    print(json.dumps({name: res[name]}), flush=True)
```

Baseline: 577,600.

## Skip MFMAs and LDS reads on zero-padded depth taps at volume edges

Remaps the wave-to-output tile layout in the direct stride-2 conv and the whole-volume transposed conv so that each wave's MFMA column tile corresponds to a single depth slab. Waves whose slab touches the zero padding at the depth boundary can then skip the corresponding ds_reads and MFMAs, with the zeroed Q registers standing in for the skipped loads. The behaviour is gated by a new VV_PAD_SKIP hook that defaults on. The change adds branchy control flow inside hand-scheduled MFMA/LDS pipelines and reorders the MFMA issue sequence, which may disturb the existing overlap or cause wave imbalance, since only edge waves skip work.

```diff
diff --git a/anytime-3d-reconstruction_amd/csrc/conv_direct.hip b/anytime-3d-reconstruction_amd/csrc/conv_direct.hip
--- a/anytime-3d-reconstruction_amd/csrc/conv_direct.hip
+++ b/anytime-3d-reconstruction_amd/csrc/conv_direct.hip
@@ -167,7 +167,7 @@
 __global__ __launch_bounds__(512, 1) void conv_direct16_kernel(const __bf16 *__restrict__ x, const __bf16 *__restrict__ w,
                                                              const float *__restrict__ scale, const float *__restrict__ shift,
                                                              void *__restrict__ y, int dout_log2, unsigned x_bytes, unsigned w_bytes,
-                                                             int act, int out_fp8) {
+                                                             int act, int out_fp8, int padskip) {
     extern __shared__ __attribute__((aligned(16))) char smem[];
     const int tid = threadIdx.x, lane = tid & 63;
     const int wave = __builtin_amdgcn_readfirstlane(tid >> 6);
@@ -214,7 +214,8 @@
     __syncthreads();
 
     const int r = lane & 15, kq = lane >> 4;
-    const int rl0 = wm * 81 + (r >> 3) * 9 + (r & 7);
+    const int rl0 = wm * 18 + (r >> 3) * 9 + (r & 7);
+    const bool edge0 = padskip && od0 == 0, edge3 = padskip && od0 + 4 == no;
     unsigned xo[2][2], wo[2];
 #pragma unroll
     for (int aw = 0; aw < 2; ++aw)
@@ -229,12 +230,12 @@
 #pragma unroll
         for (int j = 0; j < 4; ++j) acc[i][j] = f32x4{0.f, 0.f, 0.f, 0.f};
 
-#define CD16_LD(F, XA, XOFF, WA)                                                                                                    \
+#define CD16_LD(F, XA, XOFF, WA, TP)                                                                                                  \
     asm volatile("ds_read_b128 %0, %8 offset:%10\n\tds_read_b128 %1, %8 offset:%11\n\tds_read_b128 %2, %8 offset:%12\n\t"         \
                  "ds_read_b128 %3, %8 offset:%13\n\tds_read_b128 %4, %9\n\tds_read_b128 %5, %9 offset:2048\n\t"                   \
                  "ds_read_b128 %6, %9 offset:4096\n\tds_read_b128 %7, %9 offset:6144"                                               \
                  : "=&v"(F[0]), "=&v"(F[1]), "=&v"(F[2]), "=&v"(F[3]), "=&v"(F[4]), "=&v"(F[5]), "=&v"(F[6]), "=&v"(F[7])            \
-                 : "v"(XA), "v"(WA), "n"(XOFF), "n"((XOFF) + 2304), "n"((XOFF) + 4608), "n"((XOFF) + 6912)                          \
+                 : "v"(XA), "v"(WA), "n"(XOFF), "n"((XOFF) + (TP)), "n"((XOFF) + 2 * (TP)), "n"((XOFF) + 3 * (TP))                   \
                  : "memory")
 #define CD16_WAIT(F, N)                                                                                                             \
     asm volatile("s_waitcnt lgkmcnt(%8)"                                                                                            \
@@ -247,8 +248,11 @@
     acc[COT][CT] = __builtin_amdgcn_mfma_f32_16x16x32_bf16(*reinterpret_cast<const bf16x8 *>(&F[4 + COT]),                          \
                                                            *reinterpret_cast<const bf16x8 *>(&F[CT]), acc[COT][CT], 0, 0, 0)
 
+    constexpr int TP = 81 * CD_RB;
     u32x4 P[8], Q[8];
-    CD16_LD(P, xo[0][0], 0, wo[0]);
+#pragma unroll
+    for (int i = 0; i < 4; ++i) Q[i] = u32x4{0u, 0u, 0u, 0u};
+    CD16_LD(P, xo[0][0], 0, wo[0], TP);
 
 #pragma unroll 1
     for (int q = 0; q < 8; ++q) {
@@ -259,31 +263,37 @@
             constexpr int AN = (A + 1) & 7, AWN = AN & 1, TON = (((AN >> 2) & 1) * 81 + ((AN >> 1) & 1) * 9 + AWN) * CD_RB;
             const int c = q * 8 + A;
             const unsigned wsel = (c % CD_NST) * CD_WST, wnext = ((c + 1) % CD_NST) * CD_WST;
+            constexpr int TS = ((A >> 2) & 1) ? 3 : 0, TC = 3 - TS, TSN = ((AN >> 2) & 1) ? 3 : 0;
+            const bool skip = TS == 0 ? (edge0 && !(q & 4)) : (edge3 && (q & 4));
+            const bool skipn = TSN == 0 ? (edge0 && !((A == 7 ? q + 1 : q) & 4)) : (edge3 && (q & 4));
             const unsigned xq = xo[AW][1] + tsel, wq = wo[1] + wsel;
             CD16_WAIT(P, 0);
             CD16_SB;
-            CD16_MF(P, 0, 0); CD16_MF(P, 0, 1); CD16_SB; CD16_RD(Q[0], xq, TO); CD16_RD(Q[4], wq, 0); CD16_SB;
-            CD16_MF(P, 0, 2); CD16_MF(P, 0, 3); CD16_SB; CD16_RD(Q[1], xq, TO + 2304); CD16_RD(Q[5], wq, 2048); CD16_SB;
-            CD16_MF(P, 1, 0); CD16_MF(P, 1, 1); CD16_SB; CD16_RD(Q[2], xq, TO + 4608); CD16_RD(Q[6], wq, 4096); CD16_SB;
-            CD16_MF(P, 1, 2); CD16_MF(P, 1, 3); CD16_SB; CD16_RD(Q[3], xq, TO + 6912); CD16_RD(Q[7], wq, 6144); CD16_SB;
-            CD16_MF(P, 2, 0); CD16_MF(P, 2, 1); CD16_MF(P, 2, 2); CD16_MF(P, 2, 3);
-            CD16_MF(P, 3, 0); CD16_MF(P, 3, 1); CD16_MF(P, 3, 2); CD16_MF(P, 3, 3);
+            CD16_MF(P, 0, 1); CD16_MF(P, 1, 1); CD16_SB; if (TS != 0 || !skip) CD16_RD(Q[0], xq, TO); CD16_RD(Q[4], wq, 0); CD16_SB;
+            CD16_MF(P, 2, 1); CD16_MF(P, 3, 1); CD16_SB; CD16_RD(Q[1], xq, TO + TP); CD16_RD(Q[5], wq, 2048); CD16_SB;
+            CD16_MF(P, 0, 2); CD16_MF(P, 1, 2); CD16_SB; CD16_RD(Q[2], xq, TO + 2 * TP); CD16_RD(Q[6], wq, 4096); CD16_SB;
+            CD16_MF(P, 2, 2); CD16_MF(P, 3, 2); CD16_SB; if (TS != 3 || !skip) CD16_RD(Q[3], xq, TO + 3 * TP); CD16_RD(Q[7], wq, 6144); CD16_SB;
+            CD16_MF(P, 0, TC); CD16_MF(P, 1, TC); CD16_MF(P, 2, TC); CD16_MF(P, 3, TC);
+            CD16_SB;
+            if (!skip) { CD16_MF(P, 0, TS); CD16_MF(P, 1, TS); CD16_MF(P, 2, TS); CD16_MF(P, 3, TS); }
             CD16_SB;
             CD16_WAIT(Q, 0);
             vv_wait_vm<(A == 0 || A == 7) ? 2 : 3>();
             __syncthreads();
             CD16_SB;
-            CD16_MF(Q, 0, 0); CD16_MF(Q, 0, 1);
+            CD16_MF(Q, 0, 1); CD16_MF(Q, 1, 1);
             if (A < 7) issue_x(q + 1, A);
-            CD16_MF(Q, 0, 2); CD16_MF(Q, 0, 3);
+            CD16_MF(Q, 2, 1); CD16_MF(Q, 3, 1);
             issue_w(c + 3);
             const unsigned xp = xo[AWN][0] + (A == 7 ? tnext : tsel), wp = wo[0] + wnext;
             CD16_SB;
-            CD16_MF(Q, 1, 0); CD16_MF(Q, 1, 1); CD16_SB; CD16_RD(P[0], xp, TON); CD16_RD(P[4], wp, 0); CD16_SB;
-            CD16_MF(Q, 1, 2); CD16_MF(Q, 1, 3); CD16_SB; CD16_RD(P[1], xp, TON + 2304); CD16_RD(P[5], wp, 2048); CD16_SB;
-            CD16_MF(Q, 2, 0); CD16_MF(Q, 2, 1); CD16_SB; CD16_RD(P[2], xp, TON + 4608); CD16_RD(P[6], wp, 4096); CD16_SB;
-            CD16_MF(Q, 2, 2); CD16_MF(Q, 2, 3); CD16_SB; CD16_RD(P[3], xp, TON + 6912); CD16_RD(P[7], wp, 6144); CD16_SB;
-            CD16_MF(Q, 3, 0); CD16_MF(Q, 3, 1); CD16_MF(Q, 3, 2); CD16_MF(Q, 3, 3);
+            CD16_MF(Q, 0, 2); CD16_MF(Q, 1, 2); CD16_SB; if (TSN != 0 || !skipn) CD16_RD(P[0], xp, TON); CD16_RD(P[4], wp, 0); CD16_SB;
+            CD16_MF(Q, 2, 2); CD16_MF(Q, 3, 2); CD16_SB; CD16_RD(P[1], xp, TON + TP); CD16_RD(P[5], wp, 2048); CD16_SB;
+            if (!skip) { CD16_MF(Q, 0, TS); CD16_MF(Q, 1, TS); }
+            CD16_SB; CD16_RD(P[2], xp, TON + 2 * TP); CD16_RD(P[6], wp, 4096); CD16_SB;
+            if (!skip) { CD16_MF(Q, 2, TS); CD16_MF(Q, 3, TS); }
+            CD16_SB; if (TSN != 3 || !skipn) CD16_RD(P[3], xp, TON + 3 * TP); CD16_RD(P[7], wp, 6144); CD16_SB;
+            CD16_MF(Q, 0, TC); CD16_MF(Q, 1, TC); CD16_MF(Q, 2, TC); CD16_MF(Q, 3, TC);
             CD16_SB;
         };
         tap(std::integral_constant<int, 0>{});
@@ -311,7 +321,7 @@
 #pragma unroll
         for (int cot = 0; cot < 4; ++cot) shv[cot] = *reinterpret_cast<const f32x4 *>(shift + wn * 64 + cot * 16 + 4 * kq);
     }
-    auto fill = VV_DIRECT_FILL16(CD_SP, wn * 64);
+    auto fill = VV_DIRECT_FILL16(CD_SP, wn * 64, ct * 64 + wm * 16 + r);
     auto with_out = [&](auto act_c) {
         if (out_fp8) fill(act_c, std::true_type{});
         else fill(act_c, std::false_type{});
@@ -408,7 +418,7 @@
             vv_wait_vm<0>();
             __syncthreads();
         }
-        CD16_LD(P, xo[0][0], 0, wo[0] + ((q * 8) % CD_NST) * CDH_WST);
+        CD16_LD(P, xo[0][0], 0, wo[0] + ((q * 8) % CD_NST) * CDH_WST, 2304);
         auto tap = [&](auto a_c) {
             constexpr int A = decltype(a_c)::value;
             constexpr int AW = A & 1, TO = (((A >> 2) & 1) * 81 + ((A >> 1) & 1) * 9 + AW) * CD_RB;
@@ -478,7 +488,7 @@
 #pragma unroll
         for (int cot = 0; cot < 4; ++cot) shv[cot] = *reinterpret_cast<const f32x4 *>(shift + nh * CDH_COUT + cot * 16 + 4 * kq);
     }
-    auto fill = VV_DIRECT_FILL16(CDH_SP, 0);
+    auto fill = VV_DIRECT_FILL16(CDH_SP, 0, wm * 64 + ct * 16 + r);
     auto with_out = [&](auto act_c) {
         if (out_fp8) fill(act_c, std::true_type{});
         else fill(act_c, std::false_type{});
@@ -508,6 +518,7 @@
     vv_allow_lds<&conv_direct16h_kernel>(CDH_LDS);
     const int shape = vv_hook_int(vv_hook("VV_CD_SHAPE"), 16);
     const bool s16 = shape != 32, half = shape == 8;
+    const int padskip = vv_hook_int(vv_hook("VV_PAD_SKIP"), 1) != 0;
     const size_t in_per = (size_t)side * side * side * cin * 2, out_per = (size_t)so * so * so * cout * (out_dtype == VV_FP8 ? 1 : 2);
     const int per = vv_chunk_samples(in_per, batch);
     if (per < 1) return VV_ERR_SHAPE;
@@ -523,7 +534,7 @@
         else if (s16)
             VV_LAUNCH(conv_direct16_kernel, dim3(nb * boxes), dim3(512), CD_LDS, reinterpret_cast<hipStream_t>(stream), xc,
                       reinterpret_cast<const __bf16 *>(w_packed), scale, shift, yc, vv_log2(so), (unsigned)((size_t)nb * in_per),
-                      (unsigned)((size_t)64 * cin * cout * 2), act, out_dtype == VV_FP8 ? 1 : 0);
+                      (unsigned)((size_t)64 * cin * cout * 2), act, out_dtype == VV_FP8 ? 1 : 0, padskip);
         else
             VV_LAUNCH(conv_direct_kernel, dim3(nb * boxes), dim3(512), CD_LDS, reinterpret_cast<hipStream_t>(stream), xc,
                       reinterpret_cast<const __bf16 *>(w_packed), scale, shift, yc, vv_log2(so), (unsigned)((size_t)nb * in_per),
diff --git a/anytime-3d-reconstruction_amd/csrc/convt_whole.hip b/anytime-3d-reconstruction_amd/csrc/convt_whole.hip
--- a/anytime-3d-reconstruction_amd/csrc/convt_whole.hip
+++ b/anytime-3d-reconstruction_amd/csrc/convt_whole.hip
@@ -223,10 +223,12 @@
 template <int ACT, bool STATS = false>
 __global__ __launch_bounds__(512, 1) void ctw16_kernel(const __bf16 *__restrict__ x, const __bf16 *__restrict__ w,
                                                        const float *__restrict__ scale, const float *__restrict__ shift,
-                                                       __bf16 *__restrict__ y, int npar, float *__restrict__ partial = nullptr) {
+                                                       __bf16 *__restrict__ y, int npar, int padskip,
+                                                       float *__restrict__ partial = nullptr) {
     extern __shared__ __attribute__((aligned(256))) char smem[];
     const int tid = threadIdx.x, lane = tid & 63;
     const int wave = __builtin_amdgcn_readfirstlane(tid >> 6);
+    const int wd = wave >> 2, whp = wave & 3;
     const int ps = 8 / npar;
     const int b = (int)blockIdx.x / ps, p0 = ((int)blockIdx.x % ps) * npar;
     const int NC = npar * 16;
@@ -264,17 +266,17 @@
     const int r = lane & 15, q = lane >> 4;
     const int rh = r >> 3, rw = r & 7;
     const unsigned wl = lds0 + CW_RING + r * 128 + ((q ^ ((r >> 1) & 7)) << 4);
-    const unsigned R0 = lds0 + (unsigned)((wave * 64 + r) << 8);
+    const unsigned R0 = lds0 + (unsigned)((wd * 256 + (2 * whp + rh) * 8 + rw) << 8);
     const unsigned ZR = lds0 + CW_ZERO;
     auto tap_setup = [&](auto a_c, int pd, int ph, int pw, unsigned (&t)[4]) {
         constexpr int A = decltype(a_c)::value;
         const int dd = pd - ((A >> 2) & 1), dh = ph - ((A >> 1) & 1), dw = pw - (A & 1);
-        const bool okw = (unsigned)(wave + dd) < 8u && (unsigned)(rw + dw) < 8u;
+        const bool okl = (unsigned)(2 * whp + rh + dh) < 8u && (unsigned)(rw + dw) < 8u;
         const int sft = dd * 64 + dh * 8 + dw;
         const unsigned key = ((unsigned)((2 * (rw + dw)) ^ q) & 15u) << 4;
 #pragma unroll
         for (int ct = 0; ct < 4; ++ct) {
-            const unsigned row = okw && (unsigned)(2 * ct + rh + dh) < 8u ? R0 + (unsigned)((sft + 16 * ct) << 8) : ZR;
+            const unsigned row = okl && (unsigned)(4 * wd + ct + dd) < 8u ? R0 + (unsigned)((sft + 64 * ct) << 8) : ZR;
             t[ct] = row ^ key;
         }
     };
@@ -291,7 +293,7 @@
     auto epilogue = [&](int p) {
         const int pd = (p >> 2) & 1, ph = (p >> 1) & 1, pw = p & 1;
         const int qo = (q & 1) * 32 + (q >> 1) * 16;
-        char *yb = reinterpret_cast<char *>(y) + ((((size_t)b * 16 + 2 * wave + pd) * 16 + 2 * rh + ph) * 16 + 2 * rw + pw) * 128 + qo;
+        char *yb = reinterpret_cast<char *>(y) + ((((size_t)b * 16 + 8 * wd + pd) * 16 + 2 * (2 * whp + rh) + ph) * 16 + 2 * rw + pw) * 128 + qo;
         const char *ss = smem + CW_SS + q * 16;
 #pragma unroll
         for (int c2 = 0; c2 < 2; ++c2) {
@@ -320,12 +322,14 @@
             for (int ct = 0; ct < 4; ++ct) {
                 auto rx = __builtin_amdgcn_permlane16_swap(o[0][ct][0], o[1][ct][0], false, false);
                 auto ry = __builtin_amdgcn_permlane16_swap(o[0][ct][1], o[1][ct][1], false, false);
-                *reinterpret_cast<u32x4 *>(yb + (size_t)(ct * 4 * 16 * 128) + c2 * 64) = u32x4{rx[0], ry[0], rx[1], ry[1]};
+                *reinterpret_cast<u32x4 *>(yb + (size_t)(ct * 2 * 16 * 16 * 128) + c2 * 64) = u32x4{rx[0], ry[0], rx[1], ry[1]};
             }
         }
     };
 
     u32x4 P[8], Q[8];
+#pragma unroll
+    for (int i = 0; i < 4; ++i) Q[i] = u32x4{0u, 0u, 0u, 0u};
     unsigned ua[4], ub[4];
     tap_setup(std::integral_constant<int, 0>{}, (p0 >> 2) & 1, (p0 >> 1) & 1, p0 & 1, ua);
     unsigned ws = wl;
@@ -335,31 +339,37 @@
     for (int pi = 0; pi < npar; ++pi) {
         const int p = p0 + pi, pd = (p >> 2) & 1, ph = (p >> 1) & 1, pw = p & 1;
         const int pn = p + 1, pnd = (pn >> 2) & 1, pnh = (pn >> 1) & 1, pnw = pn & 1;
+        const bool sk0 = padskip && pd == 0 && wd == 0, sk3 = padskip && pd == 1 && wd == 1, skn3 = padskip && pnd == 1 && wd == 1;
         auto chunk = [&](auto j_c) {
             constexpr int J = decltype(j_c)::value, A = J >> 1, KH = J & 1;
+            constexpr int TS = ((A >> 2) & 1) ? 0 : 3, TC = 3 - TS;
+            constexpr int AN = KH ? (A + 1) & 7 : A, TSN = ((AN >> 2) & 1) ? 0 : 3;
+            const bool skip = TS == 0 ? sk0 : sk3;
+            const bool skipn = (KH && A == 7) ? skn3 : (TSN == 0 ? sk0 : sk3);
             unsigned xq[4];
 #pragma unroll
             for (int ct = 0; ct < 4; ++ct) xq[ct] = ua[ct] ^ (KH ? 192u : 64u);
             const unsigned wq = ws ^ 64u;
             CW16_WAIT(P, 0);
             CW16_SB;
-            CW16_MF(P, 0, 0); CW16_MF(P, 0, 1); CW16_SB; CW16_RD(Q[0], xq[0], 0); CW16_RD(Q[4], wq, 0); CW16_SB;
-            CW16_MF(P, 0, 2); CW16_MF(P, 0, 3); CW16_SB; CW16_RD(Q[1], xq[1], 0); CW16_RD(Q[5], wq, 2048); CW16_SB;
-            CW16_MF(P, 1, 0); CW16_MF(P, 1, 1); CW16_SB; CW16_RD(Q[2], xq[2], 0); CW16_RD(Q[6], wq, 4096); CW16_SB;
-            CW16_MF(P, 1, 2); CW16_MF(P, 1, 3); CW16_SB; CW16_RD(Q[3], xq[3], 0); CW16_RD(Q[7], wq, 6144); CW16_SB;
-            CW16_MF(P, 2, 0); CW16_MF(P, 2, 1); CW16_MF(P, 2, 2); CW16_MF(P, 2, 3);
+            CW16_MF(P, 0, 1); CW16_MF(P, 1, 1); CW16_SB; if (TS != 0 || !skip) CW16_RD(Q[0], xq[0], 0); CW16_RD(Q[4], wq, 0); CW16_SB;
+            CW16_MF(P, 2, 1); CW16_MF(P, 3, 1); CW16_SB; CW16_RD(Q[1], xq[1], 0); CW16_RD(Q[5], wq, 2048); CW16_SB;
+            CW16_MF(P, 0, 2); CW16_MF(P, 1, 2); CW16_SB; CW16_RD(Q[2], xq[2], 0); CW16_RD(Q[6], wq, 4096); CW16_SB;
+            CW16_MF(P, 2, 2); CW16_MF(P, 3, 2); CW16_SB; if (TS != 3 || !skip) CW16_RD(Q[3], xq[3], 0); CW16_RD(Q[7], wq, 6144); CW16_SB;
+            CW16_MF(P, 0, TC); CW16_MF(P, 1, TC); CW16_MF(P, 2, TC); CW16_MF(P, 3, TC);
             if (KH == 0) {
                 if (A < 7) tap_setup(std::integral_constant<int, (A + 1) & 7>{}, pd, ph, pw, ub);
                 else tap_setup(std::integral_constant<int, 0>{}, pnd, pnh, pnw, ub);
             }
-            CW16_MF(P, 3, 0); CW16_MF(P, 3, 1); CW16_MF(P, 3, 2); CW16_MF(P, 3, 3);
+            CW16_SB;
+            if (!skip) { CW16_MF(P, 0, TS); CW16_MF(P, 1, TS); CW16_MF(P, 2, TS); CW16_MF(P, 3, TS); }
             CW16_SB;
             CW16_WAIT(Q, 0);
             if (J < 2 && pi > 0) vv_wait_vm<9>();
             else vv_wait_vm<1>();
             __builtin_amdgcn_s_barrier();
             CW16_SB;
-            CW16_MF(Q, 0, 0); CW16_MF(Q, 0, 1); CW16_SB;
+            CW16_MF(Q, 0, 1); CW16_MF(Q, 1, 1); CW16_SB;
             issue_w(cw, stg);
             ++cw;
             stg = stg == CW_NST - 1 ? 0 : stg + 1;
@@ -372,12 +382,14 @@
                 for (int ct = 0; ct < 4; ++ct) xq[ct] = ua[ct] = ub[ct];
             }
             CW16_SB;
-            CW16_MF(Q, 0, 2); CW16_MF(Q, 0, 3); CW16_SB; CW16_RD(P[0], xq[0], 0); CW16_RD(P[4], ws, 0); CW16_SB;
-            CW16_MF(Q, 1, 0); CW16_MF(Q, 1, 1); CW16_SB; CW16_RD(P[1], xq[1], 0); CW16_RD(P[5], ws, 2048); CW16_SB;
-            CW16_MF(Q, 1, 2); CW16_MF(Q, 1, 3); CW16_SB; CW16_RD(P[2], xq[2], 0); CW16_RD(P[6], ws, 4096); CW16_SB;
-            CW16_MF(Q, 2, 0); CW16_MF(Q, 2, 1); CW16_SB; CW16_RD(P[3], xq[3], 0); CW16_RD(P[7], ws, 6144); CW16_SB;
-            CW16_MF(Q, 2, 2); CW16_MF(Q, 2, 3);
-            CW16_MF(Q, 3, 0); CW16_MF(Q, 3, 1); CW16_MF(Q, 3, 2); CW16_MF(Q, 3, 3);
+            CW16_MF(Q, 2, 1); CW16_MF(Q, 3, 1); CW16_SB; if (TSN != 0 || !skipn) CW16_RD(P[0], xq[0], 0); CW16_RD(P[4], ws, 0); CW16_SB;
+            CW16_MF(Q, 0, 2); CW16_MF(Q, 1, 2); CW16_SB; CW16_RD(P[1], xq[1], 0); CW16_RD(P[5], ws, 2048); CW16_SB;
+            CW16_MF(Q, 2, 2); CW16_MF(Q, 3, 2); CW16_SB; CW16_RD(P[2], xq[2], 0); CW16_RD(P[6], ws, 4096); CW16_SB;
+            if (!skip) { CW16_MF(Q, 0, TS); CW16_MF(Q, 1, TS); }
+            CW16_SB; if (TSN != 3 || !skipn) CW16_RD(P[3], xq[3], 0); CW16_RD(P[7], ws, 6144); CW16_SB;
+            if (!skip) { CW16_MF(Q, 2, TS); CW16_MF(Q, 3, TS); }
+            CW16_SB;
+            CW16_MF(Q, 0, TC); CW16_MF(Q, 1, TC); CW16_MF(Q, 2, TC); CW16_MF(Q, 3, TC);
             CW16_SB;
         };
         chunk(std::integral_constant<int, 0>{});
@@ -719,6 +731,8 @@
 
 }
 
+static int cw_pad_skip() { return vv_hook_int(vv_hook("VV_PAD_SKIP"), 1) != 0; }
+
 VV_EXPORT int vv_convT3d_k4s2_whole_supported(int side, int cin, int cout, int dtype) {
     return dtype == VV_BF16 && side == 8 && cin == 128 && cout == 64;
 }
@@ -747,7 +761,7 @@
                       reinterpret_cast<const __bf16 *>(w_skip), scale, shift, reinterpret_cast<__bf16 *>(y), 8 / ps);
         else if (shape16)
             VV_LAUNCH(ctw16_kernel<ACT>, dim3((unsigned)batch * ps), dim3(512), CW_LDS, st, reinterpret_cast<const __bf16 *>(x),
-                      reinterpret_cast<const __bf16 *>(w_skip), scale, shift, reinterpret_cast<__bf16 *>(y), 8 / ps);
+                      reinterpret_cast<const __bf16 *>(w_skip), scale, shift, reinterpret_cast<__bf16 *>(y), 8 / ps, cw_pad_skip());
         else
             VV_LAUNCH(ctw_kernel<ACT>, dim3((unsigned)batch * ps), dim3(512), CW_LDS, st, reinterpret_cast<const __bf16 *>(x),
                       reinterpret_cast<const __bf16 *>(w_skip), scale, shift, reinterpret_cast<__bf16 *>(y), 8 / ps);
@@ -767,6 +781,6 @@
     vv_allow_lds<&ctw16_kernel<VV_ACT_NONE, true>>(CW_LDS);
     VV_LAUNCH((ctw16_kernel<VV_ACT_NONE, true>), dim3((unsigned)batch), dim3(512), CW_LDS, reinterpret_cast<hipStream_t>(stream),
               reinterpret_cast<const __bf16 *>(x), reinterpret_cast<const __bf16 *>(w_skip), nullptr, nullptr, reinterpret_cast<__bf16 *>(y), 8,
-              stats_partial);
+              cw_pad_skip(), stats_partial);
     return vv_launch_status();
 }
diff --git a/anytime-3d-reconstruction_amd/csrc/direct_common.h b/anytime-3d-reconstruction_amd/csrc/direct_common.h
--- a/anytime-3d-reconstruction_amd/csrc/direct_common.h
+++ b/anytime-3d-reconstruction_amd/csrc/direct_common.h
@@ -30,7 +30,7 @@
         }                                                                                                  \
     } while (0)
 
-#define VV_DIRECT_FILL16(PITCH, C0)                                                                        \
+#define VV_DIRECT_FILL16(PITCH, C0, ROW)                                                                     \
     [&](auto act_c, auto fp8_c) {                                                                          \
         constexpr int ACT = decltype(act_c)::value;                                                        \
         constexpr bool FP8 = decltype(fp8_c)::value;                                                       \
@@ -39,7 +39,7 @@
                 const int c = (C0) + cot * 16 + 4 * kq;                                                    \
                 const f32x4 sc = scv[cot], sh = shv[cot];                                                  \
                 const f32x4 v = vv_bn_act4<ACT>(acc[cot][ct], sc, sh);                                     \
-                char *dst = stage + (wm * 64 + ct * 16 + r) * (PITCH);                                     \
+                char *dst = stage + (ROW) * (PITCH);                                                       \
                 VV_DIRECT_PUT4(dst, c, v);                                                                 \
             }                                                                                              \
     }
diff --git a/anytime-3d-reconstruction_amd/voxvae/lib.py b/anytime-3d-reconstruction_amd/voxvae/lib.py
--- a/anytime-3d-reconstruction_amd/voxvae/lib.py
+++ b/anytime-3d-reconstruction_amd/voxvae/lib.py
@@ -8,7 +8,7 @@
 HOOKS_LIB_PATH = os.path.join(PKG, 'lib', 'libvoxvae_hooks.so')
 HOOK_VARS = ('VV_CD_SHAPE', 'VV_CDH_STAGGER', 'VV_CDH_ABL', 'VV_DIRECT_MT', 'VV_LT_KSLICE', 'VV_SPLIT_TARGET', 'VV_SPLIT_MINCHUNKS', 'VV_NO_KHALVES', 'VV_POSMAJOR_CONV_SIDE',
              'VV_POSMAJOR_CONVT_SIDE', 'VV_STAGES', 'VV_NO_FIRSTCONV', 'VV_WGRAD_F32', 'VV_PG_TARGET', 'VV_CTW_PS', 'VV_CTW_SHAPE',
-             'VV_NO_WGRAD_PHASE', 'VV_BN_NB', 'VV_BN_SWEEP', 'VV_FINAL_BCE', 'VV_FIRSTCONV_GATHER', 'VV_FIRSTCONV_WGS', 'VV_FIRSTCONV_NOCHAIN', 'VV_CHUNK_SAMPLES')
+             'VV_NO_WGRAD_PHASE', 'VV_BN_NB', 'VV_BN_SWEEP', 'VV_FINAL_BCE', 'VV_FIRSTCONV_GATHER', 'VV_FIRSTCONV_WGS', 'VV_FIRSTCONV_NOCHAIN', 'VV_CHUNK_SAMPLES', 'VV_PAD_SKIP')
 
 VV_F32, VV_BF16, VV_FP8 = 0, 1, 2
 ACT = {None: 0, 'None': 0, 'linear': 0, 'elu': 1, 'relu': 2, 'lrelu': 3}
diff --git a/profiles/microbench/mb_ab_lib.py b/profiles/microbench/mb_ab_lib.py
--- a/profiles/microbench/mb_ab_lib.py
+++ b/profiles/microbench/mb_ab_lib.py
@@ -138,7 +138,7 @@
     else:
         same = bool(torch.equal(ys[other], ys['tree']))
     t = {k: [] for k in libs}
-    for rnd in range(4 if name in timed else 0):
+    for rnd in range(int(os.environ.get('AB_ROUNDS', '5')) if name in timed else 0):
         for k in libs:
             a = args(ys[k])
             for i in range(30):
```

Result: no change. 579,900, median of 6 (+0.4%).
